# fakufaku/diffusion-separation

Hardware: AMD Instinct MI355X
Metric: separated utterances/sec (4 s, 8 kHz, 2-spk, N=30 PC steps) (higher is better)
Workload: dtype f16; 1 GPU; configs[1]: 2-spk N=30 PC sampler (+1 ald2 corrector step), batch=16 x 4.0 s @ 8 kHz per GPU and step, NCSN++ nf=64 random-init, 60 NFE/step; 4 consecutive steps (batches) in flight per GPU; batch_per_gpu=16, samples=32000, N=30, corrector_steps=1, nf=64, graph=True, batches_in_flight=4

## Files before the change

### diffusion-separation_amd/csrc/common.h

```cpp
#pragma once
#include <hip/hip_runtime.h>
#include <stdint.h>
#include <stdio.h>

#include <string>

typedef uint16_t bf16_t;
typedef __attribute__((ext_vector_type(16))) float f32x16;
typedef __attribute__((ext_vector_type(8))) __bf16 bf16x8;

#define DS_F32 0
#define DS_BF16 1
#define DS_F32_SPLIT 2
#define DS_MAX_SRC 4

void ds_set_error(const std::string& s);
#define DS_CHECK(cond, msg)                                                            \
  do {                                                                                 \
    if (!(cond)) {                                                                     \
      ds_set_error(std::string(__FILE__) + ":" + std::to_string(__LINE__) + ": " + (msg)); \
      return 1;                                                                        \
    }                                                                                  \
  } while (0)
#define DS_HIP(expr)                                                                   \
  do {                                                                                 \
    hipError_t _e = (expr);                                                            \
    if (_e != hipSuccess) {                                                            \
      ds_set_error(std::string(__FILE__) + ":" + std::to_string(__LINE__) + ": " + #expr + " -> " + \
                   hipGetErrorString(_e));                                             \
      return 1;                                                                        \
    }                                                                                  \
  } while (0)
#define DS_LAUNCH_CHECK() DS_HIP(hipGetLastError())
#define DS_FUNC_LDS_ONCE(kern, bytes)                                                                              \
  do {                                                                                                             \
    static bool done_[32] = {};                                                                                    \
    int dev_ = 0;                                                                                                  \
    (void)hipGetDevice(&dev_);                                                                                     \
    if (dev_ < 0 || dev_ >= 32 || !done_[dev_]) {                                                                  \
      DS_HIP(hipFuncSetAttribute(reinterpret_cast<const void*>(kern), hipFuncAttributeMaxDynamicSharedMemorySize, (bytes))); \
      if (dev_ >= 0 && dev_ < 32) done_[dev_] = true;                                                              \
    }                                                                                                              \
  } while (0)

typedef __attribute__((ext_vector_type(2))) float f32x2_t;
typedef __attribute__((ext_vector_type(2))) __bf16 bf16x2_t;
typedef __attribute__((ext_vector_type(2))) _Float16 f16x2_t;
typedef __attribute__((ext_vector_type(8))) _Float16 f16x8;
typedef __attribute__((ext_vector_type(4))) float f32x4_acc;
__host__ __device__ inline float bf2f(bf16_t v) {
  union { uint32_t u; float f; } c; c.u = ((uint32_t)v) << 16; return c.f;
}
__device__ inline uint32_t pack_bf16x2(float lo, float hi) {
  f32x2_t v = {lo, hi};
  return __builtin_bit_cast(uint32_t, __builtin_convertvector(v, bf16x2_t));
}
__device__ inline float bf_lo(uint32_t w) { return __uint_as_float(w << 16); }
__device__ inline float bf_hi(uint32_t w) { return __uint_as_float(w & 0xffff0000u); }
__host__ __device__ inline bf16_t f2bf(float f) {
#if defined(__HIP_DEVICE_COMPILE__)
  return __builtin_bit_cast(unsigned short, (__bf16)f);
#endif
  union { uint32_t u; float f; } c; c.f = f;
  uint32_t u = c.u;
  if ((u & 0x7fffffffu) > 0x7f800000u) return (bf16_t)((u >> 16) | 0x40u);
  u += 0x7fffu + ((u >> 16) & 1u);
  return (bf16_t)(u >> 16);
}
__device__ inline f32x16 mfma_bf32(const uint4& a, const uint4& b, const f32x16& c) {
  return __builtin_amdgcn_mfma_f32_32x32x16_bf16(__builtin_bit_cast(bf16x8, a), __builtin_bit_cast(bf16x8, b), c, 0, 0, 0);
}
__device__ inline f32x4_acc mfma_bf16(const uint4& a, const uint4& b, const f32x4_acc& c) {
  return __builtin_amdgcn_mfma_f32_16x16x32_bf16(__builtin_bit_cast(bf16x8, a), __builtin_bit_cast(bf16x8, b), c, 0, 0, 0);
}
#ifdef DS_HALF_F16
#define DS_HALF_NAME "f16"
#define DS_MFMA_H32_ASM "v_mfma_f32_32x32x16_f16"
#define DS_CVT_PK_H_ASM "v_cvt_pk_f16_f32"
#define DS_H_ONE 0x3c00u
__host__ __device__ inline float h2f(bf16_t v) { return (float)__builtin_bit_cast(_Float16, v); }
__host__ __device__ inline bf16_t f2h(float f) { return __builtin_bit_cast(unsigned short, (_Float16)f); }
__device__ inline uint32_t pack_h2(float lo, float hi) {
  f32x2_t v = {lo, hi};
  return __builtin_bit_cast(uint32_t, __builtin_convertvector(v, f16x2_t));
}
__device__ inline float h_lo(uint32_t w) { return (float)__builtin_bit_cast(f16x2_t, w)[0]; }
__device__ inline float h_hi(uint32_t w) { return (float)__builtin_bit_cast(f16x2_t, w)[1]; }
__device__ inline f32x16 mfma_h32(const uint4& a, const uint4& b, const f32x16& c) {
  return __builtin_amdgcn_mfma_f32_32x32x16_f16(__builtin_bit_cast(f16x8, a), __builtin_bit_cast(f16x8, b), c, 0, 0, 0);
}
__device__ inline f32x4_acc mfma_h16(const uint4& a, const uint4& b, const f32x4_acc& c) {
  return __builtin_amdgcn_mfma_f32_16x16x32_f16(__builtin_bit_cast(f16x8, a), __builtin_bit_cast(f16x8, b), c, 0, 0, 0);
}
#else
#define DS_HALF_NAME "bf16"
#define DS_MFMA_H32_ASM "v_mfma_f32_32x32x16_bf16"
#define DS_CVT_PK_H_ASM "v_cvt_pk_bf16_f32"
#define DS_H_ONE 0x3f80u
__host__ __device__ inline float h2f(bf16_t v) { return bf2f(v); }
__host__ __device__ inline bf16_t f2h(float f) { return f2bf(f); }
__device__ inline uint32_t pack_h2(float lo, float hi) { return pack_bf16x2(lo, hi); }
__device__ inline float h_lo(uint32_t w) { return bf_lo(w); }
__device__ inline float h_hi(uint32_t w) { return bf_hi(w); }
__device__ inline f32x16 mfma_h32(const uint4& a, const uint4& b, const f32x16& c) { return mfma_bf32(a, b, c); }
__device__ inline f32x4_acc mfma_h16(const uint4& a, const uint4& b, const f32x4_acc& c) { return mfma_bf16(a, b, c); }
#endif

template <typename T> struct Elt;
template <> struct Elt<float> {
  static constexpr int KV = 4;
  __device__ static inline float ld(const float* p) { return *p; }
  __device__ static inline void st(float* p, float v) { *p = v; }
};
template <> struct Elt<bf16_t> {
  static constexpr int KV = 8;
  __device__ static inline float ld(const bf16_t* p) { return h2f(*p); }
  __device__ static inline void st(bf16_t* p, float v) { *p = f2h(v); }
};

template <typename T> __device__ inline void load8(const T* p, float* f);
template <> __device__ inline void load8<float>(const float* p, float* f) {
  float4 a = *reinterpret_cast<const float4*>(p);
  float4 b = *reinterpret_cast<const float4*>(p + 4);
  f[0] = a.x; f[1] = a.y; f[2] = a.z; f[3] = a.w; f[4] = b.x; f[5] = b.y; f[6] = b.z; f[7] = b.w;
}
template <> __device__ inline void load8<bf16_t>(const bf16_t* p, float* f) {
  uint4 u = *reinterpret_cast<const uint4*>(p);
  f[0] = h_lo(u.x); f[1] = h_hi(u.x);
  f[2] = h_lo(u.y); f[3] = h_hi(u.y);
  f[4] = h_lo(u.z); f[5] = h_hi(u.z);
  f[6] = h_lo(u.w); f[7] = h_hi(u.w);
}
template <typename T> __device__ inline void store8(T* p, const float* f);
template <> __device__ inline void store8<float>(float* p, const float* f) {
  *reinterpret_cast<float4*>(p) = make_float4(f[0], f[1], f[2], f[3]);
  *reinterpret_cast<float4*>(p + 4) = make_float4(f[4], f[5], f[6], f[7]);
}
template <> __device__ inline void store8<bf16_t>(bf16_t* p, const float* f) {
  uint4 u;
  u.x = pack_h2(f[0], f[1]);
  u.y = pack_h2(f[2], f[3]);
  u.z = pack_h2(f[4], f[5]);
  u.w = pack_h2(f[6], f[7]);
  *reinterpret_cast<uint4*>(p) = u;
}

template <typename T> __device__ inline float exp_t(float v);
template <> __device__ inline float exp_t<float>(float v) { return expf(v); }
template <> __device__ inline float exp_t<bf16_t>(float v) { return __expf(v); }
template <typename T> __device__ inline float silu_t(float v);
template <> __device__ inline float silu_t<float>(float v) { return v / (1.0f + expf(-v)); }
template <> __device__ inline float silu_t<bf16_t>(float v) { return v * __builtin_amdgcn_rcpf(1.0f + __expf(-v)); }

__device__ inline float wave_sum(float v) {
#pragma unroll
  for (int o = 32; o > 0; o >>= 1) v += __shfl_xor(v, o, 64);
  return v;
}
__device__ inline double wave_sum_d(double v) {
#pragma unroll
  for (int o = 32; o > 0; o >>= 1) v += __shfl_xor(v, o, 64);
  return v;
}
__device__ inline float wave_max(float v) {
#pragma unroll
  for (int o = 32; o > 0; o >>= 1) v = fmaxf(v, __shfl_xor(v, o, 64));
  return v;
}

static inline int cdiv(long a, long b) { return (int)((a + b - 1) / b); }

struct ConvArgs {
  const void* x; long x_bs; int ldx;
  const void* x2; long x2_bs; int ldx2;
  int C1;
  const void* w; long w_bs;
  int w_chunked;
  const void* w_frag; const void* sw_frag;
  const void* ident_frag;
  const void* sx; long sx_bs; int ldsx;
  const void* sx2; long sx2_bs; int ldsx2; int sC1; int sCin;
  const void* sw; int sw_chunked;
  const float* gn_scale;
  const float* gn_shift; int gn_act;
  const float* bias;
  const float* bias_b; int bias_b_ld;
  int bias_mode;
  const float* div_b;
  const void* res; long res_bs; int ldr;
  float out_scale;
  void* y; long y_bs; int ldy;
  long long* stats_acc;
  const long long* gn_acc1; const long long* gn_acc2; const float* gn_gamma; const float* gn_beta;
  int gn_groups; float gn_inv_count; float gn_eps;
  int B, H, W;
  int Cin, Cout, taps;
  int dtype;
  int split;
  unsigned opts;
};
#define DS_OPT_NO_RW 1u
#define DS_OPT_NO_RW128 2u
#define DS_OPT_RW_SMALL 4u
#define DS_OPT_NO_RW_RES 8u
#define DS_OPT_NO_ATTN_FUSED 64u
#define DS_OPT_NO_SPLIT256 128u
#define DS_OPT_NO_STFT_FUSED 256u
#define DS_OPT_RW_QUARTER 1024u
#define DS_OPT_RW_BIG_HALF 2048u
#define DS_OPT_RW_HALF 512u
#define DS_OPT_NO_SW 4096u
#define DS_OPT_NO_SW_RW 8192u
#define DS_OPT_NO_SW_ROWS4 32768u
#define DS_OPT_SW_ROWS4 65536u
#define DS_OPT_NO_SWS 16384u
#define DS_OPT_NO_WFRAG 32u
unsigned ds_default_opts();
int ds_num_cus();
enum { DS_CLS_CONV_N64 = 0, DS_CLS_CONV_N32, DS_CLS_CONV_8X8, DS_CLS_GEMM_N64, DS_CLS_GEMM_N32, DS_CLS_GEMM_8X8, DS_CLS_WS,
       DS_CLS_SMALL, DS_CLS_RW, DS_CLS_ATTN, DS_CLS_SW, DS_CLS_SWS, DS_NCLS };
enum class ConvRoute { GENERIC, WS, THIN_IN, THIN_OUT, SMALL, RW, SW, SWS };
struct ConvPlan {
  ConvRoute route;
  int cls;
  int tile;
  int sw_rows;
  bool rw_ok;
  bool skip_ok;
};
ConvPlan ds_conv_plan(const ConvArgs& a);
int ds_launch_conv(const ConvArgs& a, hipStream_t st);
int ds_launch_conv(const ConvArgs& a, const ConvPlan& p, hipStream_t st);
const char* ds_last_conv_kernel();
void ds_set_last_conv_kernel(const char* name);
int ds_conv_chunk(int taps, int dtype);
__host__ __device__ inline long ds_rw_frag_index(int co, int tap, int ch, int taps, int Cout) {
  return (((((long)(ch / 64) * taps + tap) * 4 + (ch % 64) / 16) * (Cout / 32) + co / 32) * 64 + ((ch % 16) / 8) * 32 + co % 32) * 8 + ch % 8;
}
inline bool ds_rw_frag_shape(int taps, int Cin, int Cout) {
  return (Cout == 64 || Cout == 128) && (Cin == 64 || Cin == 128) && (taps == 1 || !(Cout == 128 && Cin == 64));
}
bool ds_conv_rw_supported(const ConvArgs& a);
int ds_launch_conv_rw(const ConvArgs& a, hipStream_t st);
inline bool ds_sw_frag_shape(int taps, int Cin, int Cout) { return (Cout == 64 || Cout == 128 || Cout == 256) && Cin % 64 == 0 && Cin >= 64 && Cin <= 512; }
bool ds_conv_sw_supported(const ConvArgs& a);
int ds_launch_conv_sw(const ConvArgs& a, int rows, hipStream_t st);
__host__ __device__ inline long ds_sws_frag_index(int co, int tap, int ch, int taps, int Cout, int plane) {
  return ((((((long)(ch / 32) * taps + tap) * 2 + (ch % 32) / 16) * 2 + plane) * (Cout / 32) + co / 32) * 64 + ((ch % 16) / 8) * 32 + co % 32) * 8 + ch % 8;
}
inline bool ds_sws_frag_shape(int taps, int Cin, int Cout) { return (Cout == 64 || Cout == 128 || Cout == 256) && Cin % 64 == 0 && Cin >= 64 && Cin <= 256; }
bool ds_conv_sws_supported(const ConvArgs& a);
int ds_launch_conv_sws(const ConvArgs& a, hipStream_t st);
bool ds_conv_ws_supported(const ConvArgs& a);
int ds_launch_conv_ws(const ConvArgs& a, hipStream_t st);
bool ds_conv_thin_in_supported(const ConvArgs& a);
int ds_launch_conv_thin_in(const ConvArgs& a, hipStream_t st);
bool ds_conv_thin_out_supported(const ConvArgs& a);
int ds_launch_conv_thin_out(const ConvArgs& a, hipStream_t st);
bool ds_conv_small_supported(const ConvArgs& a);
int ds_launch_conv_small(const ConvArgs& a, hipStream_t st);

struct AttnFusedArgs {
  const void* x; long x_bs; int ldx;
  const long long* gn_acc; const float* gn_gamma; const float* gn_beta; int gn_groups; float gn_inv_count; float gn_eps;
  const float* gn_scale; const float* gn_shift;
  const void* wqk; const void* wv; const void* wo;
  const float* bqk; const float* bv; const float* bo;
  void* y; long y_bs; int ldy;
  long long* stats;
  int B, L, C;
};
bool ds_attn_fused_eligible(int dtype, int channels, int L);
int ds_launch_attn_fused(const AttnFusedArgs& a, hipStream_t st);

long ds_gn_workspace_bytes(int B, int H, int W, int C);
int ds_launch_gn_stats(const void* x, int ldx, const void* x2, int ldx2, int C1, int B, int H, int W, int C, int groups,
                       float eps, const float* gamma, const float* beta, void* ws, float* scale, float* shift,
                       int dtype, hipStream_t st);
int ds_launch_gn_finalize_acc(const long long* a1, int C1, const long long* a2, int C2, int B, long npix, int groups,
                              float eps, const float* gamma, const float* beta, float* scale, float* shift,
                              hipStream_t st);
int ds_launch_gn_apply(const void* x, int ldx, const float* scale, const float* shift, int C, void* y, int ldy,
                       void* xr, int ldxr, int B, int H, int W, int act, int mode, int dtype, hipStream_t st);
int ds_launch_concat(const void* a, int lda, int Ca, const void* b, int ldb, int Cb, void* y, int ldy, long npix,
                     int dtype, hipStream_t st);
int ds_launch_softmax(const void* x, void* y, long rows, int L, int ld, int dtype, hipStream_t st);

long ds_stft_workspace_bytes(int B, int S, long T, int n_fft, int hop);
long ds_istft_workspace_bytes(int B, int S, long T, int n_fft, int hop);
int ds_launch_stft_pack(const float* xt, const float* mix, void* y, int B, int S, long T, int n_fft, int hop,
                        float exponent, float factor, int W, int Cpad, int shift, int dtype, const float* tab,
                        float* ws, hipStream_t st, int split = 0);
int ds_launch_istft(const void* x, float* out, int B, int S, long T, int n_fft, int hop, float exponent, float factor,
                    int W, int Cpad, int dtype, const float* tab, float* ws, hipStream_t st, int split = 0,
                    const float* ow = nullptr, const float* ob = nullptr, const float* tdiv = nullptr, int ow_cin = 0);
int ds_build_stft_table(int n_fft, float** dev_tab);

struct SdeP { int kind; int ndim; float d_lambda, sigma_min, sigma_max; };
__device__ inline float sde_g_of_t(const SdeP& s, float t) {
  const float r = s.sigma_max / s.sigma_min;
  return s.sigma_min * powf(r, t) * sqrtf(2.0f * logf(r));
}
__device__ inline void mix_eig(const SdeP& s, float t, float& ev1, float& ev2) {
  const float r = s.sigma_max / s.sigma_min;
  const float logsig = logf(r);
  const float mult = s.sigma_min * s.sigma_min;
  const float srp = powf(r, 2.0f * t);
  ev1 = mult * (srp - 1.0f);
  const float ex = expf(-2.0f * s.d_lambda * t);
  const float denom = 1.0f + s.d_lambda / logsig;
  ev2 = mult * (srp - ex) / denom;
}
__device__ inline void philox_round(uint32_t& c0, uint32_t& c1, uint32_t& c2, uint32_t& c3, uint32_t k0, uint32_t k1) {
  const uint64_t p0 = (uint64_t)0xD2511F53u * c0;
  const uint64_t p1 = (uint64_t)0xCD9E8D57u * c2;
  const uint32_t n0 = (uint32_t)(p1 >> 32) ^ c1 ^ k0;
  const uint32_t n1 = (uint32_t)p1;
  const uint32_t n2 = (uint32_t)(p0 >> 32) ^ c3 ^ k1;
  const uint32_t n3 = (uint32_t)p0;
  c0 = n0; c1 = n1; c2 = n2; c3 = n3;
}
__device__ inline void philox_randn4(uint64_t q, uint64_t seed, uint64_t sid, float* v) {
  uint32_t c0 = (uint32_t)q, c1 = (uint32_t)(q >> 32), c2 = (uint32_t)sid, c3 = (uint32_t)(sid >> 32);
  uint32_t k0 = (uint32_t)seed, k1 = (uint32_t)(seed >> 32);
#pragma unroll
  for (int r = 0; r < 10; ++r) {
    philox_round(c0, c1, c2, c3, k0, k1);
    k0 += 0x9E3779B9u;
    k1 += 0xBB67AE85u;
  }
  const float u0 = ((float)(c0 >> 8) + 0.5f) * (1.0f / 16777216.0f);
  const float u1 = ((float)(c1 >> 8) + 0.5f) * (1.0f / 16777216.0f);
  const float u2 = ((float)(c2 >> 8) + 0.5f) * (1.0f / 16777216.0f);
  const float u3 = ((float)(c3 >> 8) + 0.5f) * (1.0f / 16777216.0f);
  const float r0 = sqrtf(-2.0f * logf(u0)), r1 = sqrtf(-2.0f * logf(u2));
  sincosf(6.28318530718f * u1, &v[1], &v[0]);
  sincosf(6.28318530718f * u3, &v[3], &v[2]);
  v[0] *= r0; v[1] *= r0; v[2] *= r1; v[3] *= r1;
}
__device__ inline void sde_mix_drift(const SdeP& s, const float* xv, float* f, int S) {
  float mx = 0.f;
  for (int i = 0; i < S; ++i) mx += xv[i];
  mx /= (float)S;
  for (int i = 0; i < S; ++i) f[i] = -s.d_lambda * (xv[i] - mx);
}
int ds_launch_sigma_mix(const float* mix, float* out, int B, long T, int avg_len, hipStream_t st);
int ds_launch_sde_prior(const SdeP& s, const float* y, const float* z, float* x, int B, int S, long T,
                        const float* smix, hipStream_t st, const int* lens = nullptr);
int ds_launch_sde_corrector(const SdeP& s, float snr, const float* x, const float* t, const float* score,
                            const float* z, float* xo, float* xm, int B, int S, long T, const float* smix,
                            int variant, hipStream_t st, const int* lens = nullptr);
int ds_launch_sde_predictor(const SdeP& s, int N, const float* x, const float* t, const float* score, const float* z,
                            float* xo, float* xm, int B, int S, long T, const float* smix, int pflow, hipStream_t st,
                            const int* lens = nullptr);
int ds_launch_sde_coeff(const SdeP& s, const float* x, const float* t, const float* smix, float* drift,
                        float* diffusion, int B, int S, long T, float fs, float gs, hipStream_t st);
int ds_launch_sde_mean(const SdeP& s, const float* x0, const float* t, float* out, int B, int S, long T, hipStream_t st);
int ds_launch_sde_std(const SdeP& s, const float* t, const float* smix, float* L, int B, int S, long T, hipStream_t st);
int ds_launch_sde_mult_std(const float* L, const float* x, float* out, int B, int S, long T, int per_t, hipStream_t st);
int ds_launch_sde_reverse(const float* f, const float* G, const float* score, float* out, int B, long n_per_batch,
                          int g_full, int pflow, hipStream_t st);
int ds_launch_randn_batch(float* out, int B, int S, long T, const uint64_t* seeds, const int* lens, uint64_t stream_id,
                          hipStream_t st);
int ds_launch_langevin(float snr, const float* x, const float* score, const float* z, float* xo, float* xm, int B,
                       long n_per_batch, void* ws, hipStream_t st);
int ds_launch_normalize(const float* mix, float* out, float* mean, float* std, int B, long T, hipStream_t st);
int ds_launch_scale_output(const float* mix, float* sep, int B, int S, long T, hipStream_t st);
int ds_launch_randn(float* out, long n, uint64_t seed, uint64_t stream_id, hipStream_t st);
int ds_launch_gram(const float* ref, const float* est, double* out, int B, int S, long T, hipStream_t st);
int ds_launch_convert(const void* src, void* dst, long n, int sd, int dd, hipStream_t st);
int ds_launch_fill(float* p, float v, long n, hipStream_t st);

#define DS_ODE_MAX_K 7
#define DS_ODE_MAX_BLOCKS 1024
int ds_ode_tableau(int method, double* A, double* B, double* C, double* E, int* n_stages, int* error_order);
struct OdeArgs {
  SdeP s;
  const float* x; const float* score; const float* tt; float t; const float* smix;
  float* kout; int kidx; int nk;
  const float* k[DS_ODE_MAX_K]; double c[DS_ODE_MAX_K];
  double h; int mode;
  const double* y; const double* ynew; double* yo; float* xo;
  double rtol, atol; double* part;
  float* t_next_out; float t_next;
  int B, S; long T;
};
int ds_launch_ode_stage(const OdeArgs& a, hipStream_t st, int* nblk = nullptr);
int ds_launch_ode_norm_final(const double* part, int nblk, long n, double* out, hipStream_t st);
int ds_launch_ode_cast(const float* x, double* y, long n, hipStream_t st);
int ds_launch_ode_round(const double* y, float* x, long n, hipStream_t st);

int ds_launch_linear(const float* x, const float* W, const float* bias, float* y, int B, int K, int O, int silu_in,
                     hipStream_t st);
int ds_launch_linear_t(const float* x, const float* Wt, const float* bias, float* y, int B, int K, int O, int silu_in,
                       hipStream_t st);
int ds_launch_dense_transpose(const float* src, float* dst, int O, int K, int ldo, int off, hipStream_t st);
int ds_launch_fourier(const float* t, const float* Wf, float* emb, int B, int nf, hipStream_t st);
```

### diffusion-separation_amd/csrc/conv3x3_rw.hip

```cpp
#include <stdlib.h>

#ifdef RW_TIMING
#define HALO_TIMING rw
#endif
#include "conv3x3_halo.h"

namespace {

constexpr int KC = 64;
constexpr int NKB = KC / 16;
constexpr int KSC = 9 * NKB;
static_assert(KC * 2 + 16 == AROW && KC / 8 == PPL, "a pixel's chunk is one 128-byte line");

struct RwK {
  const bf16_t* x; long x_bs; int ldx; int C1;
  const bf16_t* x2; long x2_bs; int ldx2;
  const bf16_t* w; int w_chunked;
  const bf16_t* wfrag; const bf16_t* swfrag;
  const float* gn_scale; const float* gn_shift;
  const long long* gn_acc1; const long long* gn_acc2; const float* gn_gamma; const float* gn_beta;
  int gn_groups; float gn_inv_count; float gn_eps;
  const float* bias; const float* bias_b; int bias_b_ld;
  const bf16_t* res; long res_bs; int ldr;
  float out_scale;
// ... 427 lines not shown
    constexpr int LAG = ACT1 ? PIPE_LAG : 0, NUV = NU + LAG, NLU = 2 * NUV;
    constexpr int NGH = NK * RH;
    constexpr int w0 = (P == 0) ? W_E : W_N, w1 = (P == NPH - 1) ? W_E : W_N, CAP = NGH * (w0 + w1);
    auto lub = [](int GP) constexpr { return NLU * (GP <= NGH ? GP * w0 : NGH * w0 + (GP - NGH) * w1) / CAP; };
    constexpr int NLE = RH * 22;
    constexpr int R0 = HF * RH, ER0 = HF ? 0 : RH;
    const char* fb = sA + slot_r * LDS_A + fbase + R0 * HW_ * AROW;
#ifndef RW_BUILTIN_MFMA
    if constexpr (EPI) {
#pragma unroll
      for (int r = 0; r < RH; ++r) asm volatile("s_nop 11" : "+v"(acc[ER0 + r]));
    }
#endif
    if constexpr (HF == 0 && C1 < NCH) act_tab(C1);
    constexpr int SUB = CONV ? 3 : 1, RFN = CONV ? RH + 2 : RH, NG = NK / SUB;
    static_assert(SUB * RH >= RFN, "the next group's fragments are read in the MFMA slots of the current one");
    auto ldg = [&](int g, int j) __attribute__((always_inline)) {
      const int dx = CONV ? g / NKB : 1, kb = g % NKB, row = CONV ? j : j + 1;
      return *reinterpret_cast<const u32x4_t*>(fb + (row * HW_ + dx) * AROW + kb * 32);
    };
    u32x4_t rf[2][RFN];
#pragma unroll
    for (int j = 0; j < RFN; ++j) rf[0][j] = ldg(0, j);
    auto widx = [](int ks) {
      if (!CONV) return ks;
      const int g = ks / 3, dy = ks % 3, dx = g / NKB, kb = g % NKB;
      return (dy * 3 + dx) * NKB + kb;
    };
#define RW_FRAG(ks, r) rf[((ks) / SUB) & 1][(r) + (CONV ? (ks) % SUB : 0)]
#define RW_FRAG_LAST(ks) rf[((ks) / SUB) & 1][RFN - 1]
    u32x4_t wl = {0, 0, 0, 0}, wln = {0, 0, 0, 0};
    if constexpr (W0 + widx(0) >= NWR) wl = *reinterpret_cast<const u32x4_t*>(sWl + (W0 + widx(0) - NWR) * G::WL_STEP);
    int rels[2][NL];
    auto fetch_rels = [&](int ks, int par) __attribute__((always_inline)) {
      const int gp0 = HF * NGH + ks * RH;
#pragma unroll
      for (int L = lub(gp0); L < lub(gp0 + RH); ++L) {
        const int u = (L >> 1) - LAG;
        if ((L & 1) && u >= 0 && u < NU && (u & 3) == 3 && (u >> 2) >= NI)
          rels[par][u >> 2] = REL_REGS ? relreg[(u >> 2) - NI] : sDesc[((u >> 2) - NI) * NT + tid];
      }
    };
    fetch_rels(0, 0);

    auto unit_lump = [&](int L, int par) __attribute__((always_inline)) {
      const int v = L >> 1;
      const int u0 = v < NU ? v : -1, u1 = LAG ? ((v >= 1 && v - 1 < NU) ? v - 1 : -1) : v, u2 = v - LAG;
      const bool s2 = u2 >= 0 && u2 < NU;
      if ((L & 1) == 0) {
        if constexpr (ACT1 && ACT_PK) {
          if (u0 >= 0) {
            asm volatile("v_pk_fma_f16 %0, %1, %2, %3" : "=v"(uzp[u0 % 3]) : "v"(pa[u0 >> 2][u0 & 3]), "v"(psc[u0 & 3]), "v"(psh[u0 & 3]));
            if constexpr (MODE == 2 && !FOLD) asm volatile("v_pk_mul_f16 %0, %1, %2" : "=v"(uxp[u0 % 3]) : "v"(uzp[u0 % 3]), "s"(0xbdc5bdc5u));
          }
          if constexpr (MODE == 2) {
            if (u1 >= 0) asm volatile("v_pk_add_f16 %0, %1, %2" : "=v"(udp[u1 % 3]) : "v"(utp[u1 % 3]), "s"(0x3c003c00u));
            if (s2) asm volatile("v_pk_mul_f16 %0, %1, %2" : "=v"(so[u2 & 3]) : "v"(uzp[u2 % 3]), "v"(urp[u2 % 3]));
            if (u0 >= 0) asm volatile("v_exp_f16 %0, %1" : "=v"(utp[u0 % 3]) : "v"(FOLD ? uzp[u0 % 3] : uxp[u0 % 3]));
            if (u1 >= 0) asm volatile("v_rcp_f16 %0, %1" : "=v"(urp[u1 % 3]) : "v"(udp[u1 % 3]));
          } else {
            if (s2) so[u2 & 3] = uzp[u2 % 3];
          }
        } else if constexpr (ACT1) {
          if (u0 >= 0) unit_s01(std::integral_constant<int, C1>{}, u0, -1);
        }
      } else {
        if constexpr (ACT1 && ACT_PK) {
          if constexpr (MODE == 2) {
            if (u0 >= 0) asm volatile("v_exp_f16_sdwa %0, %1 dst_sel:WORD_1 dst_unused:UNUSED_PRESERVE src0_sel:WORD_1" : "+v"(utp[u0 % 3]) : "v"(FOLD ? uzp[u0 % 3] : uxp[u0 % 3]));
            if (u1 >= 0) asm volatile("v_rcp_f16_sdwa %0, %1 dst_sel:WORD_1 dst_unused:UNUSED_PRESERVE src0_sel:WORD_1" : "+v"(urp[u1 % 3]) : "v"(udp[u1 % 3]));
          }
        } else if constexpr (ACT1) {
          if (u1 >= 0) unit_s01(std::integral_constant<int, C1>{}, -1, u1);
        }
#ifndef RW_ABL_NOSTAGE
        if (s2) {
          const int rel = ((u2 & 3) == 3 && (u2 >> 2) >= NI) ? rels[par][u2 >> 2] : 0;
          if constexpr (ACT1 && ACT_PK) unit_fin(std::integral_constant<int, C1>{}, std::integral_constant<int, C2>{}, g1, g2, slot_r ^ 1, u2, rel);
          else unit_s2(std::integral_constant<int, C1>{}, std::integral_constant<int, C2>{}, g1, g2, slot_r ^ 1, u2, rel);
        }
#endif
      }
    };
    auto epi_lump = [&](int LE) __attribute__((always_inline)) {
      const int rr = ER0 + LE / 22, x = LE % 22;
      if (x < 20) {
        const int j = x / 10, y = x % 10;
        const bool isA = y == 0 || y == 1 || y == 3 || y == 5 || y == 7;
        const int pr = y == 0 ? 0 : (y == 1 ? 1 : (y == 2 ? 0 : (y == 3 ? 2 : (y == 4 ? 1 : (y == 5 ? 3 : (y == 6 ? 2 : (y == 7 ? 4 : 3)))))));
        if (y == 9) {
          if (j == 0) {
            asm volatile("v_permlane32_swap_b32 %0, %1" : "+v"(osa[0]), "+v"(osa[2]));
            asm volatile("v_permlane32_swap_b32 %0, %1" : "+v"(osa[1]), "+v"(osa[3]));
          } else {
            asm volatile("v_permlane32_swap_b32 %0, %1" : "+v"(osb[0]), "+v"(osb[2]));
            asm volatile("v_permlane32_swap_b32 %0, %1" : "+v"(osb[1]), "+v"(osb[3]));
          }
        } else if (isA) {
          if (pr < 4) {
            const int e0 = 8 * j + 2 * pr;
            const float b0 = pr == 0 ? breg[j][0].x : (pr == 1 ? breg[j][0].z : (pr == 2 ? breg[j][1].x : breg[j][1].z));
            const float b1 = pr == 0 ? breg[j][0].y : (pr == 1 ? breg[j][0].w : (pr == 2 ? breg[j][1].y : breg[j][1].w));
            asm volatile("v_fma_f32 %0, %1, %2, %3" : "=v"(et[pr & 1][0]) : "v"(acc[rr][e0]), "s"(osc), "v"(b0));
            asm volatile("v_fma_f32 %0, %1, %2, %3" : "=v"(et[pr & 1][1]) : "v"(acc[rr][e0 + 1]), "s"(osc), "v"(b1));
          }
          if (pr >= 1) {
            const int q = pr - 1;
            if (j == 0) asm volatile(DS_CVT_PK_H_ASM " %0, %1, %2" : "=v"(osa[q]) : "v"(et[q & 1][0]), "v"(et[q & 1][1]));
            else asm volatile(DS_CVT_PK_H_ASM " %0, %1, %2" : "=v"(osb[q]) : "v"(et[q & 1][0]), "v"(et[q & 1][1]));
          }
        } else {
#ifndef RW_ABL_NOSTATS
          const int e0 = 8 * j + 2 * pr;
          asm volatile("v_add_f32 %0, %0, %1" : "+v"(ssum[e0]) : "v"(et[pr & 1][0]));
          asm volatile("v_add_f32 %0, %0, %1" : "+v"(ssum[e0 + 1]) : "v"(et[pr & 1][1]));
          asm volatile("v_fma_f32 %0, %1, %1, %0" : "+v"(ssq[e0]) : "v"(et[pr & 1][0]));
          asm volatile("v_fma_f32 %0, %1, %1, %0" : "+v"(ssq[e0 + 1]) : "v"(et[pr & 1][1]));
#endif
        }
      } else if (x == 20) {
#pragma unroll
        for (int d = 0; d < 4; ++d) asm volatile("v_permlane16_swap_b32 %0, %1" : "+v"(osa[d]), "+v"(osb[d]));
      } else {
        const int pix = ge.pix0 + (pg * RPW + rr) * p.W + (lane & 15);
        const unsigned o = __umul24((unsigned)pix, (unsigned)p.ldy * 2u) + spiece;
#ifdef RW_TIMING
        const unsigned o1 = (p.dbg & 1) ? OOB : o, o2 = (p.dbg & 1) ? OOB : o + 16u * (unsigned)p.ldy * 2u;
#else
        const unsigned o1 = o, o2 = o + 16u * (unsigned)p.ldy * 2u;
#endif
#ifdef RW_ABL_NOSTORE
        asm volatile("" :: "v"(osa), "v"(osb), "v"(o1), "v"(o2));
#else
        __builtin_amdgcn_raw_buffer_store_b128(osa, ry, o1, 0, 0);
        __builtin_amdgcn_raw_buffer_store_b128(osb, ry, o2, 0, 0);
#endif
      }
    };

#pragma unroll
    for (int ks = 0; ks < NK; ++ks) {
      if (ks + 1 < NK) fetch_rels(ks + 1, (ks + 1) & 1);
      const int wi = W0 + widx(ks), win = W0 + widx(ks + 1 < NK ? ks + 1 : ks);
      if (win >= NWR && ks + 1 < NK) wln = *reinterpret_cast<const u32x4_t*>(sWl + (win - NWR) * G::WL_STEP);
      const u32x4_t wk = wi < NWR ? wf[wi < NWR ? wi : 0] : wl;
#define RW_DEP , "v"(RW_FRAG_LAST(ks))
#pragma unroll
      for (int r = 0; r < RH; ++r) {
        if (wi < NWR) {
          if (P == 0 && ks == 0) asm volatile(DS_MFMA_H32_ASM " %0, %1, %2, 0" : "=v"(acc[R0 + r]) : "a"(wk), "v"(RW_FRAG(ks, r)) RW_DEP);
          else asm volatile(DS_MFMA_H32_ASM " %0, %1, %2, %0" : "+v"(acc[R0 + r]) : "a"(wk), "v"(RW_FRAG(ks, r)) RW_DEP);
        } else {
          if (P == 0 && ks == 0) asm volatile(DS_MFMA_H32_ASM " %0, %1, %2, 0" : "=v"(acc[R0 + r]) : "v"(wk), "v"(RW_FRAG(ks, r)) RW_DEP);
          else asm volatile(DS_MFMA_H32_ASM " %0, %1, %2, %0" : "+v"(acc[R0 + r]) : "v"(wk), "v"(RW_FRAG(ks, r)) RW_DEP);
        }
        {
          const int g = ks / SUB, q = (ks % SUB) * RH + r;
          if (q < RFN && g + 1 < NG) rf[(g + 1) & 1][q] = ldg(g + 1, q);
        }
        const int gh = ks * RH + r, gp = HF * NGH + gh;
#pragma unroll
        for (int L = lub(gp); L < lub(gp + 1); ++L) unit_lump(L, ks & 1);
#ifndef RW_ABL_NOEPI
        if constexpr (EPI) {
#pragma unroll
          for (int LE = gh * NLE / NGH; LE < (gh + 1) * NLE / NGH; ++LE) epi_lump(LE);
        }
#endif
      }
      wl = wln;
      __builtin_amdgcn_sched_barrier(0);
    }
  };

  TileG gc = tile_geom(0);
  constexpr int CH0 = G::chunk_of(0), CH1 = G::chunk_of(1 % NPH);
  const TileG g1st = NPH > 1 ? gc : tile_geom(1);
  {
#pragma unroll
    for (int k = 0; k < NL; ++k) issue_one(std::integral_constant<int, CH0>{}, gc, k, k < NI ? 0 : sDesc[(k < NI ? 0 : k - NI) * NT + tid]);
    load_weights();
    build_tables();
    sync_lds();
    RT_MARK(7)
    if constexpr (REL_REGS) {
#pragma unroll
      for (int k = 0; k < NB; ++k) relreg[k] = sDesc[k * NT + tid];
    }
    if constexpr (BIAS_REGS) {
#pragma unroll
      for (int j = 0; j < 2; ++j) {
        breg[j][0] = *reinterpret_cast<const float4*>(sTab + 2 * CIN + cg * 32 + 8 * (2 * j) + 4 * h);
        breg[j][1] = *reinterpret_cast<const float4*>(sTab + 2 * CIN + cg * 32 + 8 * (2 * j + 1) + 4 * h);
      }
    }
    act_tab(CH0);
#pragma unroll
    for (int u = 0; u < NL * 4; ++u)
      unit(std::integral_constant<int, CH0>{}, std::integral_constant<int, CH1>{}, gc, g1st, 0, u,
           (u >> 2) < NI ? 0 : sDesc[((u >> 2) < NI ? 0 : (u >> 2) - NI) * NT + tid]);
  }
  RT_MARK(0)
  TileG gp = tile_geom(nt);
  int ph = 0;
  TileG gnc = tile_geom(1);
  int ty2 = (t0 + 2) / p.tiles_x, tx2 = (t0 + 2) - ty2 * p.tiles_x;
  for (int i = 0; i < nt; ++i) {
    const TileG gn = gnc, gnn = geom_at(ty2, tx2, i + 2 < nt);
    auto run = [&](auto self, auto P_) __attribute__((always_inline)) {
      constexpr int P = decltype(P_)::value;
      sync_lds();
      RT_MARK(1)
      const int slot_r = ph & 1;
      half(P_, std::integral_constant<int, 0>{}, std::integral_constant<bool, P == 0>{}, slot_r, gp, ((P + 1) / NPH == 0 ? gc : gn), ((P + 2) / NPH == 0 ? gc : ((P + 2) / NPH == 1 ? gn : gnn)));
      if constexpr (P == 0) {
        if (i == 0) {
#pragma unroll
          for (int j = 0; j < 16; ++j) { ssum[j] = 0.f; ssq[j] = 0.f; }
        }
      }
      half(P_, std::integral_constant<int, 1>{}, std::integral_constant<bool, P == NPH - 1>{}, slot_r, gc, ((P + 1) / NPH == 0 ? gc : gn), ((P + 2) / NPH == 0 ? gc : ((P + 2) / NPH == 1 ? gn : gnn)));
      ++ph;
      RT_MARK(G::chunk_of(P) < NCH ? 2 : 3)
      if constexpr (P + 1 < NPH) self(self, std::integral_constant<int, P + 1>{});
    };
    run(run, std::integral_constant<int, 0>{});
    gp = gc;
    gc = gn;
    gnc = gnn;
    if (++tx2 == p.tiles_x) { tx2 = 0; ++ty2; }
  }
#ifndef RW_BUILTIN_MFMA
#pragma unroll
  for (int r = 0; r < RH; ++r) asm volatile("s_nop 11" : "+v"(acc[RH + r]));
#endif
#pragma unroll
  for (int e = 0; e < RH * 2; ++e) {
    float4 t0, t1;
    epi_bias(e & 1, t0, t1);
    epi_unit(gp, RH + (e >> 1), e & 1, t0, t1);
  }
  RT_MARK(4)
  if (has_stats) {
    __syncthreads();
    float* red = reinterpret_cast<float*>(smem);
    constexpr int RED_ROW = 36;
#pragma unroll
    for (int q = 0; q < 4; ++q) {
      *reinterpret_cast<float4*>(red + tid * RED_ROW + 4 * q) = make_float4(ssum[4 * q], ssum[4 * q + 1], ssum[4 * q + 2], ssum[4 * q + 3]);
      *reinterpret_cast<float4*>(red + tid * RED_ROW + 16 + 4 * q) = make_float4(ssq[4 * q], ssq[4 * q + 1], ssq[4 * q + 2], ssq[4 * q + 3]);
    }
    __syncthreads();
    if (tid < 2 * CO) {
      const int co = tid >> 1, st = tid & 1;
      const int wcg = co >> 5, c32 = co & 31, q = c32 >> 3, hh = (c32 >> 2) & 1, i = c32 & 3;
      double a = 0.0;
      for (int wpg = 0; wpg < PGN; ++wpg)
        for (int l = 0; l < 32; ++l) {
          const int t = (wpg * NCG + wcg) * 64 + hh * 32 + l;
          a += (double)red[t * RED_ROW + st * 16 + 4 * q + i];
        }
      ds_stat_flush(p.stats + ((long)b * CO + co) * 2, st, a);
    }
  }
  RT_MARK(5)
  RT_FLUSH
}

int rw_blocks_per_image(const ConvArgs& a, int tiles) {
  int g = ds_num_cus() / a.B;
#ifdef RW_TIMING
  if (getenv("DIFFSEP_RW_G")) g = atoi(getenv("DIFFSEP_RW_G"));
#endif
  if ((a.opts & DS_OPT_RW_HALF) && g >= 2 && tiles / g <= 4) g /= 2;
  if ((a.opts & DS_OPT_RW_QUARTER) && g >= 4 && tiles / g <= 4) g /= 4;
  if ((a.opts & DS_OPT_RW_BIG_HALF) && g >= 2 && tiles / g > 4) g /= 2;
  if (g < 1) g = 1;
  if (g > tiles) g = tiles;
  return g;
}

template <int NCH, int RPW, int NSK, int MODE, int NCG>
int rw_launch(const RwK& k0, const ConvArgs& a, hipStream_t st) {
  using G = RwGeom<NCH, RPW, NSK, NCG>;
  RwK k = k0;
  const int tiles = (a.H / G::TH) * (a.W / TW);
  k.G = rw_blocks_per_image(a, tiles);
  k.tiles_x = a.W / TW;
  k.tiles_per_img = tiles;
  auto kern = conv3x3_rw_kernel<NCH, RPW, NSK, MODE, NCG>;
  DS_FUNC_LDS_ONCE(kern, G::LDS_TOTAL);
  hipLaunchKernelGGL(kern, dim3(a.B * k.G), dim3(NT), G::LDS_TOTAL, st, k);
  DS_LAUNCH_CHECK();
  {
    static char name[64] = {0};
    if (!name[0]) snprintf(name, sizeof(name), "conv3x3_rw_kernel<%d,%d,%d,%d,%d>", NCH, RPW, NSK, MODE, NCG);
    ds_set_last_conv_kernel(name);
  }
  return 0;
}

}

bool ds_conv_rw_supported(const ConvArgs& a) {
  const int CO = a.Cout;
  if (!(a.dtype == DS_BF16 && a.taps == 9 && ((CO == 64 && (a.Cin == 64 || a.Cin == 128)) || (CO == 128 && a.Cin == 128)) &&
        a.w_bs == 0 && (a.w_chunked == 0 || a.w_chunked == 32) && a.bias_mode == 0 && !a.div_b && a.W % TW == 0 && a.H % 8 == 0 &&
        a.H >= 32 && a.W >= 32 && a.ldy >= CO && a.ldy % 8 == 0 && (!a.res || (a.ldr >= CO && a.ldr % 8 == 0))))
    return false;
  if (a.x2 ? !(a.C1 % KC == 0 && a.C1 > 0 && a.C1 < a.Cin && a.ldx % 8 == 0 && a.ldx2 % 8 == 0) : a.ldx % 8 != 0) return false;
  const bool gn = a.gn_scale || a.gn_acc1;
  if (gn && !a.gn_act) return false;
  if (a.gn_acc1 && !(a.gn_groups > 0 && a.Cin % a.gn_groups == 0 && a.Cin / a.gn_groups <= 8 && (!a.x2 || a.gn_acc2))) return false;
  if (a.sx) {
    if (!(a.sw && !a.res && (a.sCin == 64 || a.sCin == 128 || (a.sCin == 192 && CO == 64 && a.Cin == 64)) && a.ldsx % 8 == 0 &&
          (!a.sx2 || (a.sC1 % KC == 0 && a.sC1 > 0 && a.sC1 < a.sCin && a.ldsx2 % 8 == 0)) &&
          (a.sw_chunked == 0 || ((a.sw_chunked & (a.sw_chunked - 1)) == 0 && a.sw_chunked >= 16))))
      return false;
    if (a.Cin == 128 && CO == 64) return false;
  }
  if (a.res && a.Cin == 128 && CO == 64) return false;
  if (CO == 128 && (a.sx || a.res) && !gn) return false;
  return true;
}

int ds_launch_conv_rw(const ConvArgs& a, hipStream_t st) {
  RwK k;
  k.x = reinterpret_cast<const bf16_t*>(a.x); k.x_bs = a.x_bs; k.ldx = a.ldx; k.C1 = a.x2 ? a.C1 : a.Cin;
  k.x2 = reinterpret_cast<const bf16_t*>(a.x2); k.x2_bs = a.x2_bs; k.ldx2 = a.x2 ? a.ldx2 : a.ldx;
  k.w = reinterpret_cast<const bf16_t*>(a.w); k.w_chunked = a.w_chunked;
  k.wfrag = reinterpret_cast<const bf16_t*>(a.w_frag);
  k.swfrag = (a.sx && a.sw) ? reinterpret_cast<const bf16_t*>(a.sw_frag) : nullptr;
  k.gn_scale = a.gn_scale; k.gn_shift = a.gn_shift;
  k.gn_acc1 = a.gn_acc1; k.gn_acc2 = a.gn_acc2; k.gn_gamma = a.gn_gamma; k.gn_beta = a.gn_beta;
  k.gn_groups = a.gn_groups; k.gn_inv_count = a.gn_inv_count; k.gn_eps = a.gn_eps;
  k.bias = a.bias; k.bias_b = a.bias_b; k.bias_b_ld = a.bias_b_ld;
  k.res = reinterpret_cast<const bf16_t*>(a.res); k.res_bs = a.res_bs; k.ldr = a.ldr;
  k.out_scale = a.out_scale;
  k.y = reinterpret_cast<bf16_t*>(a.y); k.y_bs = a.y_bs; k.ldy = a.ldy;
  k.stats = a.stats_acc;
  k.sx = reinterpret_cast<const bf16_t*>(a.sx); k.sx_bs = a.sx_bs; k.ldsx = a.ldsx; k.sC1 = a.sx2 ? a.sC1 : a.sCin;
  k.sx2 = reinterpret_cast<const bf16_t*>(a.sx2); k.sx2_bs = a.sx2_bs; k.ldsx2 = a.sx2 ? a.ldsx2 : a.ldsx;
  k.sw = reinterpret_cast<const bf16_t*>(a.sw); k.sw_chunked = a.sw_chunked; k.sw_shift = a.sw_chunked ? __builtin_ctz(a.sw_chunked) : 0;
  k.sCin = a.sCin;
  k.H = a.H; k.W = a.W; k.G = 0; k.tiles_x = 0; k.tiles_per_img = 0;
#ifdef RW_TIMING
  k.dbg = getenv("DIFFSEP_RW_DBG") ? atoi(getenv("DIFFSEP_RW_DBG")) : 0;
#else
  k.dbg = 0;
#endif
  if (a.res) {
    k.sx = reinterpret_cast<const bf16_t*>(a.res); k.sx_bs = a.res_bs; k.ldsx = a.ldr; k.sC1 = a.Cout;
    k.sx2 = nullptr; k.sx2_bs = 0; k.ldsx2 = a.ldr; k.sw = nullptr; k.sw_chunked = 0; k.sw_shift = 0; k.sCin = a.Cout;
  }
  const int mode = ((a.gn_scale || a.gn_acc1) && a.gn_act) ? 2 : 0;
  const int nsk = a.sx ? a.sCin / KC : (a.res ? a.Cout / KC : 0);
  if (a.Cout == 128) {
    if (mode == 0) return rw_launch<2, 4, 0, 0, 4>(k, a, st);
    if (nsk == 0) return rw_launch<2, 4, 0, 2, 4>(k, a, st);
    if (nsk == 1) return rw_launch<2, 4, 1, 2, 4>(k, a, st);
    return rw_launch<2, 4, 2, 2, 4>(k, a, st);
  }
#define RW_GO(NCH_, NSK_) return mode == 2 ? rw_launch<NCH_, 4, NSK_, 2, 2>(k, a, st) : rw_launch<NCH_, 4, NSK_, 0, 2>(k, a, st)
  if (a.Cin == 128) RW_GO(2, 0);
  if (nsk == 0) RW_GO(1, 0);
  if (nsk == 1) RW_GO(1, 1);
  if (nsk == 2) RW_GO(1, 2);
  RW_GO(1, 3);
#undef RW_GO
}
```

### diffusion-separation_amd/csrc/conv_mfma.hip

```cpp
#include <stdlib.h>
#include <string.h>

#include <type_traits>

#include "conv_device.h"

#ifdef CONV_TIMING
__device__ unsigned long long g_conv_dbg[16];
#define CT_DECL unsigned long long ct_prev = __builtin_readcyclecounter(), ct_acc[12] = {0, 0, 0, 0, 0, 0, 0, 0, 0, 0, 0, 0};
#define CT_MARK(i) { unsigned long long ct_now = __builtin_readcyclecounter(); ct_acc[i] += ct_now - ct_prev; ct_prev = ct_now; }
#define CT_WAIT __builtin_amdgcn_s_waitcnt(0);
#define CT_FLUSH if (threadIdx.x == 0) { for (int q = 0; q < 12; ++q) atomicAdd(&g_conv_dbg[q], ct_acc[q]); atomicAdd(&g_conv_dbg[15], 1ull); }
extern "C" int diffsep_debug_read(unsigned long long* out, int reset) {
  (void)hipMemcpyFromSymbol(out, HIP_SYMBOL(g_conv_dbg), sizeof(unsigned long long) * 16);
  if (reset) { unsigned long long z[16] = {0}; (void)hipMemcpyToSymbol(HIP_SYMBOL(g_conv_dbg), z, sizeof(z)); }
  return 0;
}
#else
#define CT_DECL
#define CT_MARK(i)
#define CT_WAIT
#define CT_FLUSH
#endif

// ... 474 lines not shown
      } else {
        if (c + 1 < ncht) load_chunk(c + 1);
        CT_MARK(5)
        mma_chunk(std::false_type{}, std::false_type{});
      }
      CT_MARK(6)
    }
    if constexpr (SKIP_OK) {
      for (int c = nch; c < ncht; ++c) {
        __syncthreads();
        write_chunk(true);
        __syncthreads();
        if (c + 1 < ncht) load_chunk(c + 1);
        mma_chunk(std::false_type{}, std::true_type{});
      }
    }
  };
  if (!has_gn) run_chunks(std::integral_constant<int, 0>{});
  else if (p.gn_act) run_chunks(std::integral_constant<int, 2>{});
  else run_chunks(std::integral_constant<int, 1>{});

  const __amdgpu_buffer_rsrc_t ry =
      rsrc(reinterpret_cast<T*>(p.y) + (long)b * p.y_bs, (unsigned)M * p.ldy * ESZ);
  const __amdgpu_buffer_rsrc_t rr = rsrc(
      p.res ? reinterpret_cast<const T*>(p.res) + (long)b * p.res_bs : reinterpret_cast<const T*>(p.y),
      p.res ? (unsigned)M * p.ldr * ESZ : 0u);
#ifdef ABL_NOEPI
  {
    float t = 0.f;
#pragma unroll
    for (int i = 0; i < WM; ++i)
#pragma unroll
      for (int j = 0; j < WN; ++j)
#pragma unroll
        for (int r = 0; r < 16; ++r) t += acc[i][j][r];
    if (t == 12345.678f) reinterpret_cast<float*>(p.y)[tid] = t;
    return;
  }
#endif
  const int cout8 = (p.Cout + 7) & ~7;
  const float dvs = p.div_b ? p.div_b[b] : 1.0f;
  constexpr int NCG = BN / 8;
  static_assert(NT % NCG == 0, "a thread keeps one cout group across the epilogue loop");
  constexpr int WME = WM / EP;
  constexpr int RV = ESZ * 8 / 16;
  const int cg = tid % NCG;
  const int co = n0 + cg * 8;
  float bv[8];
  {
    float b1[8], b2[8];
    const float* pb1 = (p.bias_mode == 0 && p.bias) ? p.bias : nullptr;
    const float* pb2 = (p.bias_mode == 0 && p.bias_b) ? p.bias_b + (long)b * p.bias_b_ld : nullptr;
#pragma unroll
    for (int j = 0; j < 8; ++j) {
      const int cc = (co + j < p.Cout) ? co + j : p.Cout - 1;
      b1[j] = pb1 ? pb1[cc] : 0.f;
      b2[j] = pb2 ? pb2[cc] : 0.f;
    }
#pragma unroll
    for (int j = 0; j < 8; ++j) bv[j] = (co + j < p.Cout) ? b1[j] + b2[j] : 0.f;
#pragma unroll
    for (int j = 0; j < 8; ++j) asm volatile("" : "+v"(bv[j]));
  }
  const bool overhang = (TAPS == 9) ? (y0 + TH > p.H || x0 + TW > p.W) : (m0 + BM > M);
  const bool lean = p.bias_mode == 0 && !p.div_b && !overhang && n0 + BN <= cout8;
  float ssum[8], ssq[8];
#pragma unroll
  for (int j = 0; j < 8; ++j) { ssum[j] = 0.f; ssq[j] = 0.f; }
#pragma unroll
  for (int e = 0; e < EP; ++e) {
    __syncthreads();
#pragma unroll
    for (int i = 0; i < WME; ++i)
#pragma unroll
      for (int j = 0; j < WN; ++j)
#pragma unroll
        for (int g = 0; g < 4; ++g) {
          const int lp = (wm * WME + i) * 32 + l32;
          const int cc = (wn * WN + j) * 32 + 8 * g + 4 * h;
          *reinterpret_cast<float4*>(smem + lp * OROW + cc * 4) =
              make_float4(acc[e * WME + i][j][4 * g], acc[e * WME + i][j][4 * g + 1], acc[e * WME + i][j][4 * g + 2],
                          acc[e * WME + i][j][4 * g + 3]);
        }
    constexpr int NROW = (BM / EP) / (NT / NCG);
    static_assert((BM / EP) % (NT / NCG) == 0, "whole rows per thread");
    int mrow[NROW];
    unsigned voy[NROW], vor[NROW];
    uint4 rraw[NROW][RV];
    constexpr int RSTEP = NT / NCG;
    const int pp0 = tid / NCG;
    const int gy0 = y0 + pp0 / TW, gx0 = x0 + pp0 % TW;
    const int mlin0 = (TAPS == 9) ? gy0 * p.W + gx0 : m0 + pp0;
    const int mstep = (TAPS == 9) ? (RSTEP / TW) * p.W : RSTEP;
    const bool col_ok = co < cout8 && (TAPS != 9 || gx0 < p.W);
#pragma unroll
    for (int it = 0; it < NROW; ++it) {
      int m = -1;
      if (EP == 1 && (TAPS != 9 || RSTEP % TW == 0)) {
        const bool ok = col_ok && ((TAPS == 9) ? (gy0 + it * (RSTEP / TW) < p.H) : (mlin0 + it * mstep < M));
        m = ok ? mlin0 + it * mstep : -1;
      } else {
        const int lp = tid / NCG + it * (NT / NCG);
        const int pp = ((lp / (32 * WME)) * WM + e * WME + (lp / 32) % WME) * 32 + (lp & 31);
        if (TAPS == 9) {
          const int gy = y0 + pp / TW, gx = x0 + pp % TW;
          if (gy < p.H && gx < p.W) m = gy * p.W + gx;
        } else {
          if (m0 + pp < M) m = m0 + pp;
        }
        if (co >= cout8) m = -1;
      }
      mrow[it] = m;
      voy[it] = m >= 0 ? (unsigned)(m * p.ldy + co) * ESZ : OOB;
      vor[it] = m >= 0 ? (unsigned)(m * p.ldr + co) * ESZ : OOB;
#pragma unroll
      for (int q = 0; q < RV; ++q) rraw[it][q] = ld16(rr, vor[it], 16u * q);
    }
    __syncthreads();
    CT_MARK(7)
    uint4 oraw[NROW][RV];
    if (lean) {
      const float osc = p.out_scale;
      float bs[8];
#pragma unroll
      for (int j = 0; j < 8; ++j) bs[j] = bv[j] * osc;
      const bool has_res = p.res != nullptr, has_stats = p.stats != nullptr;
#pragma unroll
      for (int it = 0; it < NROW; ++it) {
        const int lp = tid / NCG + it * (NT / NCG);
        const float4 a0 = *reinterpret_cast<const float4*>(smem + lp * OROW + cg * 32);
        const float4 a1 = *reinterpret_cast<const float4*>(smem + lp * OROW + cg * 32 + 16);
        float v[8] = {a0.x, a0.y, a0.z, a0.w, a1.x, a1.y, a1.z, a1.w};
#pragma unroll
        for (int j = 0; j < 8; ++j) v[j] = fmaf(v[j], osc, bs[j]);
        if (has_res) {
          float rv[8];
          unpack8<T>(rraw[it], rv);
#pragma unroll
          for (int j = 0; j < 8; ++j) v[j] = fmaf(rv[j], osc, v[j]);
        }
        if (has_stats) {
#pragma unroll
          for (int j = 0; j < 8; ++j) {
            ssum[j] += v[j];
            ssq[j] = fmaf(v[j], v[j], ssq[j]);
          }
        }
        pack8<T>(v, oraw[it]);
      }
    } else {
#pragma unroll
      for (int it = 0; it < NROW; ++it) {
        const int m = mrow[it];
        const int lp = tid / NCG + it * (NT / NCG);
        float v[8];
        const float4 a0 = *reinterpret_cast<const float4*>(smem + lp * OROW + cg * 32);
        const float4 a1 = *reinterpret_cast<const float4*>(smem + lp * OROW + cg * 32 + 16);
        v[0] = a0.x; v[1] = a0.y; v[2] = a0.z; v[3] = a0.w; v[4] = a1.x; v[5] = a1.y; v[6] = a1.z; v[7] = a1.w;
        float rv[8];
        unpack8<T>(rraw[it], rv);
        if (p.div_b) {
#pragma unroll
          for (int j = 0; j < 8; ++j) v[j] = v[j] / dvs;
        }
        if (p.bias_mode == 1 && p.bias) {
          const float rowb = p.bias[m < 0 ? 0 : m];
#pragma unroll
          for (int j = 0; j < 8; ++j) v[j] = (co + j < p.Cout) ? v[j] + rowb : 0.f;
        }
#pragma unroll
        for (int j = 0; j < 8; ++j) v[j] = (v[j] + bv[j] + rv[j]) * p.out_scale;
        const float keep = m < 0 ? 0.f : 1.f;
#pragma unroll
        for (int j = 0; j < 8; ++j) {
          ssum[j] = fmaf(keep, v[j], ssum[j]);
          asm volatile("" : "+v"(ssum[j]));
          ssq[j] = fmaf(keep * v[j], v[j], ssq[j]);
          asm volatile("" : "+v"(ssq[j]));
        }
        pack8<T>(v, oraw[it]);
      }
    }
    CT_MARK(8)
#pragma unroll
    for (int it = 0; it < NROW; ++it)
#pragma unroll
      for (int q = 0; q < RV; ++q) buf_store16(ry, voy[it], 16u * q, oraw[it][q]);
    CT_MARK(9)
  }
  if (p.stats) {
    __syncthreads();
    float* sr = reinterpret_cast<float*>(smem);
    const int r = tid / NCG;
#pragma unroll
    for (int j = 0; j < 8; ++j) {
      sr[(r * BN + cg * 8 + j) * 2 + 0] = ssum[j];
      sr[(r * BN + cg * 8 + j) * 2 + 1] = ssq[j];
    }
    __syncthreads();
    if (tid < BN && n0 + tid < p.Cout) {
      double a = 0.0, q = 0.0;
      for (int rr2 = 0; rr2 < NT / NCG; ++rr2) {
        a += (double)sr[(rr2 * BN + tid) * 2 + 0];
        q += (double)sr[(rr2 * BN + tid) * 2 + 1];
      }
      long long* o = p.stats + ((long)b * p.Cout + n0 + tid) * 2;
      ds_stat_add(o, (long long)llrint(a * DS_STAT_SUM_SCALE));
      ds_stat_add(o + 1, (long long)llrint(q * DS_STAT_SQ_SCALE));
    }
  }
  CT_MARK(10)
  CT_FLUSH
}

template <typename T, int TAPS, int TH, int TW, int BN, int WM, int WN, int KC, int EP = 1, int OCC = 2, int SP = 0, int NT = 256>
static int launch_cfg(const ConvArgs& a, hipStream_t st) {
  using G = ConvGeom<T, TAPS, TH, TW, BN, KC, EP, NT>;
  constexpr int LDS = G::LDS + 4096;
  auto kern = conv_mfma_kernel<T, TAPS, TH, TW, BN, WM, WN, KC, EP, OCC, SP, NT>;
  DS_FUNC_LDS_ONCE(kern, LDS);
  ConvK k;
  k.x = a.x; k.x_bs = a.x_bs; k.ldx = a.ldx; k.C1 = a.x2 ? a.C1 : a.Cin;
  k.x2 = a.x2; k.x2_bs = a.x2_bs; k.ldx2 = a.ldx2;
  k.w = a.w; k.w_bs = a.w_bs;
  DS_CHECK(a.w_chunked == 0 || (a.w_chunked >= 8 && KC % a.w_chunked == 0 && a.Cin % KC == 0 && (!a.x2 || a.C1 % KC == 0)),
           "conv: chunk-major weights need kc | the kernel's chunk width and whole chunks per source");
  k.w_chunked = a.w_chunked; k.w_shift = a.w_chunked ? __builtin_ctz(a.w_chunked) : 0;
  DS_CHECK((a.w_chunked & (a.w_chunked - 1)) == 0 && (a.sw_chunked & (a.sw_chunked - 1)) == 0, "conv: weight chunks are powers of two");
  DS_CHECK(!a.sx || (G::SKIP_OK && a.sw && a.sCin % 8 == 0 && a.ldsx % 8 == 0 &&
                     (a.sw_chunked == 0 || (a.sw_chunked >= 8 && KC % a.sw_chunked == 0 && a.sCin % KC == 0 &&
                                            (!a.sx2 || a.sC1 % KC == 0)))),
           "conv: bad fused skip convolution arguments");
  k.sx = a.sx; k.sx_bs = a.sx_bs; k.ldsx = a.ldsx; k.sx2 = a.sx2; k.sx2_bs = a.sx2_bs; k.ldsx2 = a.ldsx2;
  k.sC1 = a.sx2 ? a.sC1 : a.sCin; k.sCin = a.sCin; k.sw = a.sw; k.sw_chunked = a.sw_chunked; k.sw_shift = a.sw_chunked ? __builtin_ctz(a.sw_chunked) : 0;
  k.gn_scale = a.gn_scale; k.gn_shift = a.gn_shift; k.gn_act = a.gn_act;
  k.bias = a.bias; k.bias_b = a.bias_b; k.bias_b_ld = a.bias_b_ld; k.bias_mode = a.bias_mode; k.div_b = a.div_b;
  k.res = a.res; k.res_bs = a.res_bs; k.ldr = a.ldr; k.out_scale = a.out_scale;
  k.y = a.y; k.y_bs = a.y_bs; k.ldy = a.ldy; k.stats = a.stats_acc;
  k.gn_acc1 = a.gn_acc1; k.gn_acc2 = a.gn_acc2; k.gn_gamma = a.gn_gamma; k.gn_beta = a.gn_beta;
  k.gn_groups = a.gn_groups; k.gn_inv_count = a.gn_inv_count; k.gn_eps = a.gn_eps;
  DS_CHECK(!a.gn_acc1 || (a.Cin <= 512 && a.gn_groups > 0 && a.Cin % a.gn_groups == 0 && (!a.x2 || a.gn_acc2)),
           "conv: bad GroupNorm accumulator arguments");
  k.H = a.H; k.W = a.W; k.Cin = a.Cin; k.Cout = a.Cout;
  dim3 grid;
  if (TAPS == 9) {
    k.tiles_x = cdiv(a.W, TW);
    grid.x = k.tiles_x * cdiv(a.H, TH);
  } else {
    k.tiles_x = 1;
    grid.x = cdiv((long)a.H * a.W, TH * TW);
  }
  grid.y = cdiv(a.Cout, BN);
  grid.z = a.B;
  hipLaunchKernelGGL(kern, grid, dim3(NT), LDS, st, k);
  DS_LAUNCH_CHECK();
  {
    static char name[128] = {0};
    if (!name[0])
      snprintf(name, sizeof(name), "conv_mfma_kernel<%s,%d,%d,%d,%d,%d,%d,%d,%d,%d,%d,%d>", sizeof(T) == 2 ? DS_HALF_NAME : "float", TAPS,
               TH, TW, BN, WM, WN, KC, EP, OCC, SP, NT);
    ds_set_last_conv_kernel(name);
  }
  return 0;
}

static thread_local const char* g_last_conv_kernel = "";
const char* ds_last_conv_kernel() { return g_last_conv_kernel; }
void ds_set_last_conv_kernel(const char* name) { g_last_conv_kernel = name; }

template <typename T, int SP = 0>
static int launch_typed(const ConvArgs& a, int tile, hipStream_t st) {
  constexpr int KC9 = (sizeof(T) == 4) ? 16 : 32;
  constexpr int KC1 = (sizeof(T) == 4) ? 32 : 64;
  switch (tile) {
    case DS_CLS_CONV_N64: {
      const long blocks = (long)cdiv(a.W, 32) * cdiv(a.H, 8) * cdiv(a.Cout, 64) * a.B;
      if constexpr (sizeof(T) == 2) {
      if (blocks <= 128) return launch_cfg<T, 9, 8, 16, 64, 1, 2, KC9, 1, 2, SP>(a, st);
      if (!a.sx && a.Cin >= 128 && a.Cout == 64 && a.H % 16 == 0 && blocks >= 1024)
        return launch_cfg<T, 9, 16, 32, 64, 2, 2, KC9, 2, 2, SP, 512>(a, st);
      if (a.Cout % 128 == 0 && blocks >= 1024)
        return launch_cfg<T, 9, 8, 32, 128, 2, 2, KC9, 2, 2, SP, 512>(a, st);
      }
      return launch_cfg<T, 9, 8, 32, 64, 2, 2, KC9, 1, 2, SP>(a, st);
    }
    case DS_CLS_CONV_N32: return launch_cfg<T, 9, 8, 32, 32, 2, 1, KC9, 1, 2, SP>(a, st);
    case DS_CLS_CONV_8X8: {
      const bool deep = a.Cin % (2 * KC9) == 0 && (!a.x2 || a.C1 % (2 * KC9) == 0) &&
                        (!a.sx || (a.sCin % (2 * KC9) == 0 && (!a.sx2 || a.sC1 % (2 * KC9) == 0)));
      if (deep) return launch_cfg<T, 9, 8, 8, 64, 1, 1, KC9 * 2, 1, 2, SP>(a, st);
      return launch_cfg<T, 9, 8, 8, 64, 1, 1, KC9, 1, 2, SP>(a, st);
    }
    case DS_CLS_GEMM_N64: return launch_cfg<T, 1, 8, 32, 64, 2, 2, KC1, 1, 2, SP>(a, st);
    case DS_CLS_GEMM_N32: return launch_cfg<T, 1, 8, 32, 32, 2, 1, KC1, 1, 2, SP>(a, st);
    default: return launch_cfg<T, 1, 8, 8, 64, 1, 1, KC1, 1, 2, SP>(a, st);
  }
}

int ds_conv_chunk(int taps, int dtype) {
  if (dtype == DS_F32) return taps == 9 ? 16 : 32;
  return taps == 9 ? 32 : 64;
}

ConvPlan ds_conv_plan(const ConvArgs& a) {
  const unsigned o = a.opts;
  const bool any_size = o & DS_OPT_RW_SMALL;
  const long cus = ds_num_cus(), ncb = a.Cout >= 128 ? a.Cout / 128 : 1;
  const long t8 = (long)a.B * (a.H / 8) * (a.W / 32) * ncb, t4 = (long)a.B * (a.H / 4) * (a.W / 32) * ncb;
  ConvPlan p = {ConvRoute::GENERIC, -1, -1, 0, false, false};
  auto routed = [&](ConvRoute r, int cls) {
    p.route = r; p.cls = cls; p.tile = r == ConvRoute::GENERIC ? cls : -1; p.skip_ok = a.taps == 9 && cls != DS_CLS_CONV_N32;
    return p;
  };
  if (!(o & DS_OPT_NO_SWS) && ds_conv_sws_supported(a) && (2 * (a.Cout == 64 ? t8 : t4) >= cus || any_size))
    return routed(ConvRoute::SWS, DS_CLS_SWS);
  p.rw_ok = !(o & DS_OPT_NO_RW) && ds_conv_rw_supported(a) &&
            (a.Cout == 128 ? !(o & DS_OPT_NO_RW128) && (t4 >= cus || any_size)
                           : !(a.res && (o & DS_OPT_NO_RW_RES)) && (t8 >= cus || any_size));
  if (ds_conv_sw_supported(a)) {
    const bool rows8 = a.H % 8 == 0 && !(o & DS_OPT_SW_ROWS4);
    const int rows = a.Cout == 64 ? 4 : rows8 && (t4 >= 2 * cus || any_size) ? 8 : (2 * t4 >= cus || any_size) ? 4 : 0;
    p.sw_rows = rows ? rows : (rows8 ? 8 : 4);
    const bool take = a.Cout == 64 ? t8 >= cus || any_size
                                   : rows && !(rows == 4 && (o & DS_OPT_NO_SW_ROWS4)) && (!p.rw_ok || (!(o & DS_OPT_NO_SW_RW) && t8 < 2 * cus));
    if (take && !(o & DS_OPT_NO_SW)) return routed(ConvRoute::SW, DS_CLS_SW);
  }
  if (p.rw_ok) return routed(ConvRoute::RW, DS_CLS_RW);
  if (ds_conv_ws_supported(a)) return routed(ConvRoute::WS, DS_CLS_WS);
  if (ds_conv_thin_in_supported(a)) return routed(ConvRoute::THIN_IN, DS_CLS_WS);
  if (ds_conv_thin_out_supported(a)) return routed(ConvRoute::THIN_OUT, DS_CLS_WS);
  if (ds_conv_small_supported(a)) return routed(ConvRoute::SMALL, DS_CLS_SMALL);
  if (a.taps == 9)
    return routed(ConvRoute::GENERIC, !(a.W >= 32 && a.H >= 8) ? DS_CLS_CONV_8X8 : a.Cout <= 32 ? DS_CLS_CONV_N32 : DS_CLS_CONV_N64);
  if ((long)a.H * a.W >= 1024 || ((long)a.H * a.W >= 256 && a.Cout >= 1024))
    return routed(ConvRoute::GENERIC, a.Cout <= 32 ? DS_CLS_GEMM_N32 : DS_CLS_GEMM_N64);
  return routed(ConvRoute::GENERIC, DS_CLS_GEMM_8X8);
}

int ds_launch_conv(const ConvArgs& a, hipStream_t st) { return ds_launch_conv(a, ds_conv_plan(a), st); }
int ds_launch_conv(const ConvArgs& a, const ConvPlan& p, hipStream_t st) {
  DS_CHECK(a.taps == 1 || a.taps == 9, "conv: taps must be 1 or 9");
  DS_CHECK(a.Cin % 8 == 0 && a.ldx % 8 == 0, "conv: Cin and ldx must be multiples of 8");
  DS_CHECK(a.B > 0 && a.H > 0 && a.W > 0 && a.Cout > 0, "conv: empty problem");
  DS_CHECK(a.x && a.w && a.y, "conv: null pointer");
  DS_CHECK(a.ldy >= ((a.Cout + 7) & ~7), "conv: output pixel stride must cover Cout rounded up to 8");
  DS_CHECK(!a.x2 || (a.C1 % 8 == 0 && a.C1 > 0 && a.C1 < a.Cin && a.ldx2 % 8 == 0), "conv: bad concat split");
  {
    const long esz = a.dtype == DS_F32 ? 4 : 2, M = (long)a.H * a.W;
    long mld = a.ldx > a.ldy ? a.ldx : a.ldy;
    if (a.x2 && a.ldx2 > mld) mld = a.ldx2;
    if (a.res && a.ldr > mld) mld = a.ldr;
    DS_CHECK(M * mld * esz < 2147483647L, "conv: image too large for 32-bit buffer offsets");
    DS_CHECK((long)a.Cout * a.taps * a.Cin * esz < 2147483647L, "conv: weight tensor too large");
  }
  switch (p.route) {
    case ConvRoute::SWS: return ds_launch_conv_sws(a, st);
    case ConvRoute::SW: return ds_launch_conv_sw(a, p.sw_rows, st);
    case ConvRoute::RW: return ds_launch_conv_rw(a, st);
    case ConvRoute::WS: return ds_launch_conv_ws(a, st);
    case ConvRoute::THIN_IN: return ds_launch_conv_thin_in(a, st);
    case ConvRoute::THIN_OUT: return ds_launch_conv_thin_out(a, st);
    case ConvRoute::SMALL: return ds_launch_conv_small(a, st);
    case ConvRoute::GENERIC: break;
  }
  if (a.dtype == DS_F32) return a.split ? launch_typed<float, 1>(a, p.tile, st) : launch_typed<float, 0>(a, p.tile, st);
  if (a.dtype == DS_BF16) return launch_typed<bf16_t>(a, p.tile, st);
  DS_CHECK(false, "conv: unknown dtype");
}
```

### diffusion-separation_amd/csrc/engine.hip

```cpp
#include "engine_host.h"

static thread_local std::string g_err;
void ds_set_error(const std::string& s) { g_err = s; }
extern "C" const char* diffsep_last_error(void) { return g_err.c_str(); }
extern "C" const char* diffsep_version(void) {
#ifdef DS_HALF_F16
    return "diffsep-hip 0.3 (gfx950, 16-bit storage f16)";
#else
    return "diffsep-hip 0.3 (gfx950, 16-bit storage bf16)";
#endif
}

static const struct { const char* name; const char* env; unsigned bit; } kOpts[] = {
    {"no_rw", "DIFFSEP_NO_RW", DS_OPT_NO_RW},
    {"no_rw128", "DIFFSEP_NO_RW128", DS_OPT_NO_RW128},
    {"rw_small", "DIFFSEP_RW_SMALL", DS_OPT_RW_SMALL},
    {"no_rw_res", "DIFFSEP_NO_RW_RES", DS_OPT_NO_RW_RES},
    {"no_wfrag", nullptr, DS_OPT_NO_WFRAG},
    {"no_attn_fused", nullptr, DS_OPT_NO_ATTN_FUSED},
    {"no_stft_fused", "DIFFSEP_NO_STFT_FUSED", DS_OPT_NO_STFT_FUSED},
    {"rw_half", "DIFFSEP_RW_HALF", DS_OPT_RW_HALF},
    {"rw_quarter", "DIFFSEP_RW_QUARTER", DS_OPT_RW_QUARTER},
    {"rw_big_half", "DIFFSEP_RW_BIG_HALF", DS_OPT_RW_BIG_HALF},
    {"no_split256", nullptr, DS_OPT_NO_SPLIT256},
    {"no_sw", "DIFFSEP_NO_SW", DS_OPT_NO_SW},
    {"no_sws", "DIFFSEP_NO_SWS", DS_OPT_NO_SWS},
    {"no_sw_rows4", "DIFFSEP_NO_SW_ROWS4", DS_OPT_NO_SW_ROWS4},
    {"sw_rows4", nullptr, DS_OPT_SW_ROWS4},
    {"no_sw_rw", "DIFFSEP_NO_SW_RW", DS_OPT_NO_SW_RW}};
static std::atomic<unsigned> g_opts{0};
static std::once_flag g_opts_once;
unsigned ds_default_opts() {
  std::call_once(g_opts_once, [] {
    for (const auto& o : kOpts) {
      const char* v = o.env ? getenv(o.env) : nullptr;
      if (v && *v && strcmp(v, "0") != 0) g_opts |= o.bit;
    }
  });
  return g_opts;
}
int ds_num_cus() {
  static std::atomic<int> cus[32];
  int dev = 0;
  if (hipGetDevice(&dev) != hipSuccess || dev < 0 || dev >= 32) dev = 0;
  int c = cus[dev].load(std::memory_order_relaxed);
  if (c <= 0) {
    hipDeviceProp_t prop;
    c = hipGetDeviceProperties(&prop, dev) == hipSuccess ? prop.multiProcessorCount : 0;
    if (c <= 0) c = 256;
    cus[dev].store(c, std::memory_order_relaxed);
  }
  return c;
}
static int opt_bit(const char* name, unsigned* bit) {
  for (const auto& o : kOpts)
    if (!strcmp(name, o.name)) { *bit = o.bit; return 0; }
  return 1;
}
extern "C" int32_t diffsep_set_option(const char* name, int64_t value) {
  DS_CHECK(name, "set_option: null name");
  unsigned bit = 0;
  if (opt_bit(name, &bit)) { ds_set_error(std::string("set_option: unknown option '") + name + "'"); return 1; }
  ds_default_opts();
  if (value) g_opts.fetch_or(bit); else g_opts.fetch_and(~bit);
  return 0;
}

static Tn cat_view(const Tn& a, const Tn& b) {
  Tn t = a;
  t.C = a.C + b.C; t.C1 = a.C; t.p2 = b.p; t.ld2 = b.ld;
  t.sa2 = b.sa;
  return t;
}

static void* e_alloc(diffsep_engine* e, size_t bytes) {
  const size_t a = (e->top + 255) & ~(size_t)255;
  e->top = a + bytes;
  if (e->dry) return (void*)(uintptr_t)(a + 256);
  if (e->dbg_alloc) fprintf(stderr, "[diffsep alloc] %zu %zu\n", a, bytes);
  return e->arena + a;
}
static long long* e_alloc_stats(diffsep_engine* e, size_t bytes) {
  const size_t a = (e->stats_used + 255) & ~(size_t)255;
  e->stats_used = a + bytes;
  if (e->dry) { if (e->stats_used > e->stats_need) e->stats_need = e->stats_used; return (long long*)(uintptr_t)256; }
  if (e->stats_used > e->stats_need) { ds_set_error("internal: GroupNorm accumulator region overflow"); return nullptr; }
  return (long long*)(e->stats_ptr + a);
}
int stats_begin(diffsep_engine* e, hipStream_t st) {
  e->stats_used = 0;
  if (e->dry) { e->stats_need = 0; return 0; }
  e->stats_ptr = (char*)e_alloc(e, e->stats_need);
  if (e->stats_need && ds_launch_fill((float*)e->stats_ptr, 0.f, (long)(e->stats_need / 4), st)) return 1;
  return 0;
}
static Tn e_tensor(diffsep_engine* e, int B, int H, int W, int C) {
  Tn t;
  t.C = C; t.ld = C; t.H = H; t.W = W;
  t.p = e_alloc(e, (size_t)B * H * W * C * e->esz);
  if (e->track_tensors && !e->dry) e->tracked.push_back({t.p, (long)B * H * W * C, H, W, C});
  return t;
}
float* e_f32(diffsep_engine* e, size_t n) { return (float*)e_alloc(e, n * 4); }
static const float* P(diffsep_engine* e, const PRef& r) { return e->d_blob + r.off; }
static const void* PK(diffsep_engine* e, long off) { return e->d_pack + off * e->esz; }
static const void* PKF(diffsep_engine* e, long off) { return off >= 0 ? e->d_pack + off * e->esz : nullptr; }

static bool ablated(const diffsep_engine* e, int H) {
  if (!e->ablate) return false;
  const unsigned bit = H <= 16 ? 1u : H == 32 ? 2u : H == 64 ? 4u : H == 128 ? 32u : H == 256 ? 64u : 0u;
  return (e->ablate & bit) != 0;
}

struct GnAff {
  float* scale = nullptr; float* shift = nullptr;
  const long long* acc1 = nullptr; const long long* acc2 = nullptr;
  const float* gamma = nullptr; const float* beta = nullptr; int groups = 0; float inv_count = 0.f;
};
struct SkipConv { const Tn* x; const void* w; int chunk; const void* w_frag; };
struct Conv {
  const Tn& x;
  const void* w;
  int Cout, taps;
  Conv(const Tn& x_, const void* w_, int Cout_, int taps_) : x(x_), w(w_), Cout(Cout_), taps(taps_) {}
  const void* w_frag = nullptr;
  const void* ident_frag = nullptr;
  const float* bias = nullptr;
  const float* bias_b = nullptr;
  int bias_b_ld = 0;
  const float* div_b = nullptr;
  const Tn* res = nullptr;
  float scale = 1.f;
  const GnAff* gn = nullptr;
  const SkipConv* skip = nullptr;
  bool want_stats = false;
};
static ConvArgs conv_args(const diffsep_engine* e, const Conv& c, const Tn& y, int B) {
  const Tn& x = c.x;
  ConvArgs a;
  memset(&a, 0, sizeof(a));
  a.B = B; a.Cout = c.Cout; a.taps = c.taps; a.dtype = e->cfg.dtype; a.split = e->split; a.opts = e->opts;
  conv_input(a, x);
  if (c.gn) {
    a.gn_scale = c.gn->scale; a.gn_shift = c.gn->shift; a.gn_act = 1;
    if (c.gn->acc1) {
      a.gn_acc1 = c.gn->acc1; a.gn_acc2 = c.gn->acc2; a.gn_gamma = c.gn->gamma; a.gn_beta = c.gn->beta;
      a.gn_groups = c.gn->groups; a.gn_inv_count = c.gn->inv_count; a.gn_eps = 1e-6f;
    }
  }
  a.w = c.w; a.w_bs = 0; a.w_chunked = weight_chunk(c.taps, x.C, x.p2 ? x.C1 : 0, e->cfg.dtype);
  const bool use_frag = (e->cfg.dtype == DS_BF16 || (e->cfg.dtype == DS_F32 && e->split)) && !(e->opts & DS_OPT_NO_WFRAG);
  a.w_frag = use_frag ? c.w_frag : nullptr;
  a.ident_frag = use_frag ? c.ident_frag : nullptr;
  a.bias = c.bias; a.bias_b = c.bias_b; a.bias_b_ld = c.bias_b_ld; a.bias_mode = 0; a.div_b = c.div_b;
  if (c.res) conv_residual(a, *c.res);
  a.out_scale = c.scale;
  conv_output(a, y);
  if (c.skip) {
    conv_skip_input(a, *c.skip->x);
    a.sw = c.skip->w; a.sw_chunked = c.skip->chunk;
    a.sw_frag = use_frag ? c.skip->w_frag : nullptr;
  }
  return a;
}
static int conv(diffsep_engine* e, const Conv& c, Tn& y, int B, hipStream_t st) {
  ConvArgs a = conv_args(e, c, y, B);
  if (c.want_stats) {
    y.sa = e_alloc_stats(e, (size_t)B * c.Cout * 2 * sizeof(long long));
    if (!y.sa) return 1;
    a.stats_acc = y.sa;
  }
  const ConvPlan p = ds_conv_plan(a);
  DS_CHECK(!a.sx || p.skip_ok, "internal: fused skip conv on an unsupported tile");
  if (c.want_stats && e->dbg_alloc && !e->dry)
    fprintf(stderr, "[diffsep stats] %ld Cin %d Cout %d taps %d HxW %dx%d res %d skip %d bias_b %d cfg %d\n",
            (long)((char*)y.sa - e->stats_ptr), a.Cin, c.Cout, c.taps, a.H, a.W, c.res != nullptr, c.skip != nullptr,
            c.bias_b != nullptr, p.cls);
  if (e->dry || ablated(e, a.H)) return 0;
  if (!e->prof) return ds_launch_conv(a, p, st);
  diffsep_engine::ProfRec r;
  r.flops = 2.0 * ((double)a.taps * a.Cin + (a.sx ? a.sCin : 0)) * a.Cout * (double)a.H * a.W * a.B;
  {
    const double esz = a.dtype == DS_F32 ? 4.0 : 2.0;
    r.bytes = esz * ((double)a.B * a.H * a.W *
                         ((double)a.Cin + a.Cout + (a.res ? a.Cout : 0) + (a.sx ? a.sCin : 0)) +
                     ((double)a.taps * a.Cin + (a.sx ? a.sCin : 0)) * a.Cout);
  }
  r.cls = p.cls;
  r.B = a.B; r.H = a.H; r.W = a.W; r.Cin = a.Cin; r.Cout = a.Cout; r.taps = a.taps; r.sCin = a.sx ? a.sCin : 0; r.res = a.res != nullptr;
  const int rc = prof_launch(e, st, r, [&]() { return ds_launch_conv(a, p, st); });
  e->prof_recs.back().kernel = ds_last_conv_kernel();
  return rc;
}

static int gn_stats(diffsep_engine* e, const Tn& x, const float* gamma, const float* beta, int B, GnAff& aff,
                    hipStream_t st, bool lazy = false) {
  const int groups = gn_group_count(x.C);
  aff = GnAff();
  const bool have_acc = x.sa && (!x.p2 || x.sa2);
  if (have_acc && lazy && x.C <= 512) {
    aff.acc1 = x.sa; aff.acc2 = x.sa2; aff.gamma = gamma; aff.beta = beta; aff.groups = groups;
    aff.inv_count = gn_inv_count((long)x.H * x.W, x.C, groups);
    return 0;
  }
  aff.scale = e_f32(e, (size_t)B * x.C);
  aff.shift = e_f32(e, (size_t)B * x.C);
  if (have_acc) {
    if (e->dry || (e->ablate & 16u)) return 0;
    return ds_launch_gn_finalize_acc(x.sa, x.p2 ? x.C1 : x.C, x.sa2, x.p2 ? x.C - x.C1 : 0, B, (long)x.H * x.W, groups,
                                     1e-6f, gamma, beta, aff.scale, aff.shift, st);
  }
  void* ws = e_alloc(e, (size_t)ds_gn_workspace_bytes(B, x.H, x.W, x.C));
  if (e->dry) return 0;
  return ds_launch_gn_stats(x.p, x.ld, x.p2, x.ld2, x.C1, B, x.H, x.W, x.C, groups, 1e-6f, gamma, beta, ws, aff.scale,
                            aff.shift, e->cfg.dtype, st);
}
static int gn_apply(diffsep_engine* e, const Tn& x, const GnAff* aff, const Tn* y, const Tn* xr, int B, int act,
                    int mode, hipStream_t st) {
  if (e->dry || (e->ablate & 8u)) return 0;
  const double esz = e->cfg.dtype == DS_F32 ? 4.0 : 2.0, nin = (double)B * x.H * x.W * x.C;
  const double fo = mode == 1 ? 4.0 : (mode == 2 ? 0.25 : 1.0);
  const double bytes = esz * nin * (1.0 + fo * ((y ? 1 : 0) + (xr ? 1 : 0)));
  const char* name = mode == 1 ? (aff ? "gn_fir_up (GroupNorm + SiLU + FIR x2 up of act and raw)" : "fir_up (pyramid)")
                               : (mode == 2 ? (aff ? "gn_fir_down (GroupNorm + SiLU + FIR x2 down of act and raw)" : "fir_down (pyramid)")
                                            : "gn_apply (GroupNorm affine + SiLU)");
  return prof_launch(e, st, hbm_rec(name, bytes, B, x.H, x.W, x.C), [&]() {
    return ds_launch_gn_apply(x.p, x.ld, aff ? aff->scale : nullptr, aff ? aff->shift : nullptr, x.C, y ? y->p : nullptr,
                              y ? y->ld : 0, xr ? xr->p : nullptr, xr ? xr->ld : 0, B, x.H, x.W, act, mode, e->cfg.dtype,
                              st);
  });
}

static const float kInvSqrt2 = 0.70710678118654752440f;

static int conv1_folded_skip(diffsep_engine* e, const Module& m, const Tn& h1, const Tn& skip_src, const GnAff& a1, Tn& out,
                             int B, hipStream_t st) {
  const SkipConv sk = {&skip_src, PK(e, m.pk2), weight_chunk(9, m.in_ch, m.in_c1, e->cfg.dtype), PKF(e, m.pf2)};
  Conv c(h1, PK(e, m.pk1), m.out_ch, 9);
  c.w_frag = PKF(e, m.pf1); c.gn = &a1; c.skip = &sk; c.scale = kInvSqrt2; c.want_stats = true;
  c.bias = P(e, m.conv1_b); c.bias_b = P(e, m.conv2_b);
  return conv(e, c, out, B, st);
}

int res_block(diffsep_engine* e, const Module& m, const Tn& x, const float* temb_proj, int B, Tn& out,
              hipStream_t st) {
  DS_CHECK(x.C == m.in_ch, "internal: resblock channel mismatch");
  const int mode = m.up ? 1 : (m.down ? 2 : 0);
  const int Ho = m.up ? 2 * x.H : (m.down ? x.H / 2 : x.H);
  const int Wo = m.up ? 2 * x.W : (m.down ? x.W / 2 : x.W);
  GnAff a0, a1;
  const float* temb = temb_proj + m.temb_off;
  if (e->cfg.dtype == DS_BF16 && mode == 0 && x.p2 && m.pf0a >= 0 && x.C1 == 128 && x.sa && x.sa2 &&
      x.H >= ((e->opts & DS_OPT_NO_SW) ? 128 : 256) && !(e->opts & (DS_OPT_NO_SPLIT256 | DS_OPT_NO_WFRAG))) {
    Tn xa = x, xb = x;
    xa.C = 128; xa.p2 = nullptr; xa.C1 = 0; xa.ld2 = 0; xa.sa2 = nullptr;
    xb.p = x.p2; xb.ld = x.ld2; xb.C = 128; xb.p2 = nullptr; xb.C1 = 0; xb.ld2 = 0; xb.sa = x.sa2; xb.sa2 = nullptr;
    GnAff ga, gb;
    ga.acc1 = xa.sa; ga.gamma = P(e, m.gn0_w); ga.beta = P(e, m.gn0_b);
    ga.groups = gn_group_count(x.C) / 2;
    ga.inv_count = gn_inv_count((long)x.H * x.W, x.C, gn_group_count(x.C));
    gb = ga; gb.acc1 = xb.sa; gb.gamma = ga.gamma + 128; gb.beta = ga.beta + 128;
    Conv c0a(xa, PK(e, m.pk0), m.out_ch, 9);
    c0a.w_frag = PKF(e, m.pf0a); c0a.gn = &ga; c0a.bias = P(e, m.conv0_b); c0a.bias_b = temb; c0a.bias_b_ld = e->arch.dense_total;
    Tn h1p; h1p.C = h1p.ld = m.out_ch; h1p.H = Ho; h1p.W = Wo;
    ConvArgs half = conv_args(e, c0a, h1p, B); half.opts &= ~DS_OPT_RW_SMALL;
    if (ds_conv_plan(half).rw_ok) {
      h1p = e_tensor(e, B, Ho, Wo, m.out_ch);
      Tn h1 = e_tensor(e, B, Ho, Wo, m.out_ch);
      const long half0 = 4L * 9 * m.out_ch * 32;
      if (conv(e, c0a, h1p, B, st)) return 1;
      Conv c0b(xb, PK(e, m.pk0 + half0), m.out_ch, 9);
      c0b.w_frag = PKF(e, m.pf0b); c0b.gn = &gb; c0b.res = &h1p; c0b.want_stats = true;
      if (conv(e, c0b, h1, B, st)) return 1;
      if (gn_stats(e, h1, P(e, m.gn1_w), P(e, m.gn1_b), B, a1, st, true)) return 1;
      out = e_tensor(e, B, Ho, Wo, m.out_ch);
      if (!(e->opts & DS_OPT_NO_SW) && m.pf2 >= 0) return conv1_folded_skip(e, m, h1, x, a1, out, B, st);
      Tn outp = e_tensor(e, B, Ho, Wo, m.out_ch);
      const SkipConv sk = {&xa, PK(e, m.pk2), weight_chunk(9, 128, 0, e->cfg.dtype), PKF(e, m.pf2a)};
      Conv c1(h1, PK(e, m.pk1), m.out_ch, 9);
      c1.w_frag = PKF(e, m.pf1); c1.gn = &a1; c1.skip = &sk; c1.bias = P(e, m.conv1_b); c1.bias_b = P(e, m.conv2_b);
      if (conv(e, c1, outp, B, st)) return 1;
      Conv c2b(xb, PK(e, m.pk2b), m.out_ch, 1);
      c2b.res = &outp; c2b.scale = kInvSqrt2; c2b.want_stats = true;
      return conv(e, c2b, out, B, st);
    }
  }
  if (gn_stats(e, x, P(e, m.gn0_w), P(e, m.gn0_b), B, a0, st, mode == 0)) return 1;
  Tn h1 = e_tensor(e, B, Ho, Wo, m.out_ch);
  Tn xr = x, h0m;
  if (mode) {
    DS_CHECK(x.p2 == nullptr, "internal: resampling block on a concat view");
    h0m = e_tensor(e, B, Ho, Wo, m.in_ch);
    xr = e_tensor(e, B, Ho, Wo, m.in_ch);
    if (gn_apply(e, x, &a0, &h0m, &xr, B, 1, mode, st)) return 1;
  }
  if (!m.has_conv2) DS_CHECK(xr.p2 == nullptr, "internal: identity skip on a concat view");
  Conv c0(mode ? h0m : x, PK(e, m.pk0), m.out_ch, 9);
  c0.w_frag = PKF(e, m.pf0); c0.gn = mode ? nullptr : &a0; c0.want_stats = true;
  c0.bias = P(e, m.conv0_b); c0.bias_b = temb; c0.bias_b_ld = e->arch.dense_total;
  if (conv(e, c0, h1, B, st)) return 1;
  if (gn_stats(e, h1, P(e, m.gn1_w), P(e, m.gn1_b), B, a1, st, true)) return 1;
  out = e_tensor(e, B, Ho, Wo, m.out_ch);
  if (m.has_conv2 && fuse_skip(m)) return conv1_folded_skip(e, m, h1, xr, a1, out, B, st);
  Tn skip = xr;
  if (m.has_conv2) {
    skip = e_tensor(e, B, Ho, Wo, m.out_ch);
    Conv c2(xr, PK(e, m.pk2), m.out_ch, 1);
    c2.bias = P(e, m.conv2_b);
    if (conv(e, c2, skip, B, st)) return 1;
  }
  Conv c1(h1, PK(e, m.pk1), m.out_ch, 9);
  c1.w_frag = PKF(e, m.pf1); c1.ident_frag = m.has_conv2 ? nullptr : PKF(e, m.pf_id);
  c1.gn = &a1; c1.bias = P(e, m.conv1_b); c1.res = &skip; c1.scale = kInvSqrt2; c1.want_stats = true;
  return conv(e, c1, out, B, st);
}

int attention_core(const Tn& q, const void* k, const void* vt, const Tn& o, int B, void* scores, void* probs, int dtype,
                   hipStream_t st, int split) {
  const int L = q.W, C = q.C, Lp = rup8(L);
  Tn s = q, p = q;
// ... 552 lines not shown
```

Baseline: 76.02 utterances/s.

## Add 512-thread RW2 conv3x3 kernel variant and widen RW eligibility to short images

Adds a new 64->64 channel 3x3 convolution kernel (RW2) that uses 512 threads per block. It stages eight-row tiles and splits weight fragments between registers and LDS. The kernel is wired into the conv planner behind an off-by-default flag, so it only runs when the rw2_all option is set. Separately, the existing RW kernel now accepts Cout=64 layers with image height down to 8 rather than 32. That routes the low-resolution U-Net levels onto the register-weight path instead of the generic or other routes. This routing change is active by default and risks worse occupancy on tiny images.

Measured after the change: 75.88 utterances/s. Within noise of the previous version (-0.2%).

```diff
diff --git a/diffusion-separation_amd/csrc/common.h b/diffusion-separation_amd/csrc/common.h
--- a/diffusion-separation_amd/csrc/common.h
+++ b/diffusion-separation_amd/csrc/common.h
@@ -214,12 +214,14 @@
 #define DS_OPT_NO_SW_ROWS4 32768u
 #define DS_OPT_SW_ROWS4 65536u
 #define DS_OPT_NO_SWS 16384u
+#define DS_OPT_NO_RW2 131072u
+#define DS_OPT_RW2_ALL 262144u
 #define DS_OPT_NO_WFRAG 32u
 unsigned ds_default_opts();
 int ds_num_cus();
 enum { DS_CLS_CONV_N64 = 0, DS_CLS_CONV_N32, DS_CLS_CONV_8X8, DS_CLS_GEMM_N64, DS_CLS_GEMM_N32, DS_CLS_GEMM_8X8, DS_CLS_WS,
        DS_CLS_SMALL, DS_CLS_RW, DS_CLS_ATTN, DS_CLS_SW, DS_CLS_SWS, DS_NCLS };
-enum class ConvRoute { GENERIC, WS, THIN_IN, THIN_OUT, SMALL, RW, SW, SWS };
+enum class ConvRoute { GENERIC, WS, THIN_IN, THIN_OUT, SMALL, RW, SW, SWS, RW2 };
 struct ConvPlan {
   ConvRoute route;
   int cls;
@@ -242,6 +244,9 @@
 }
 bool ds_conv_rw_supported(const ConvArgs& a);
 int ds_launch_conv_rw(const ConvArgs& a, hipStream_t st);
+int ds_rw_blocks_per_image(const ConvArgs& a, int tiles);
+bool ds_conv_rw2_supported(const ConvArgs& a);
+int ds_launch_conv_rw2(const ConvArgs& a, hipStream_t st);
 inline bool ds_sw_frag_shape(int taps, int Cin, int Cout) { return (Cout == 64 || Cout == 128 || Cout == 256) && Cin % 64 == 0 && Cin >= 64 && Cin <= 512; }
 bool ds_conv_sw_supported(const ConvArgs& a);
 int ds_launch_conv_sw(const ConvArgs& a, int rows, hipStream_t st);
diff --git a/diffusion-separation_amd/csrc/conv3x3_rw.hip b/diffusion-separation_amd/csrc/conv3x3_rw.hip
--- a/diffusion-separation_amd/csrc/conv3x3_rw.hip
+++ b/diffusion-separation_amd/csrc/conv3x3_rw.hip
@@ -753,11 +753,13 @@
 
 }
 
+int ds_rw_blocks_per_image(const ConvArgs& a, int tiles) { return rw_blocks_per_image(a, tiles); }
+
 bool ds_conv_rw_supported(const ConvArgs& a) {
   const int CO = a.Cout;
   if (!(a.dtype == DS_BF16 && a.taps == 9 && ((CO == 64 && (a.Cin == 64 || a.Cin == 128)) || (CO == 128 && a.Cin == 128)) &&
         a.w_bs == 0 && (a.w_chunked == 0 || a.w_chunked == 32) && a.bias_mode == 0 && !a.div_b && a.W % TW == 0 && a.H % 8 == 0 &&
-        a.H >= 32 && a.W >= 32 && a.ldy >= CO && a.ldy % 8 == 0 && (!a.res || (a.ldr >= CO && a.ldr % 8 == 0))))
+        a.H >= (CO == 64 ? 8 : 32) && a.W >= 32 && a.ldy >= CO && a.ldy % 8 == 0 && (!a.res || (a.ldr >= CO && a.ldr % 8 == 0))))
     return false;
   if (a.x2 ? !(a.C1 % KC == 0 && a.C1 > 0 && a.C1 < a.Cin && a.ldx % 8 == 0 && a.ldx2 % 8 == 0) : a.ldx % 8 != 0) return false;
   const bool gn = a.gn_scale || a.gn_acc1;
diff --git a/diffusion-separation_amd/csrc/conv3x3_rw2.hip b/diffusion-separation_amd/csrc/conv3x3_rw2.hip
--- /dev/null
+++ b/diffusion-separation_amd/csrc/conv3x3_rw2.hip
@@ -0,0 +1,748 @@
+#include <stdlib.h>
+
+#include "conv3x3_halo.h"
+
+namespace {
+
+constexpr int KC = 64;
+constexpr int NKB = KC / 16;
+constexpr int KSC = 9 * NKB;
+static_assert(KC * 2 + 16 == AROW && KC / 8 == PPL, "a pixel's chunk is one 128-byte line");
+
+struct RwK {
+  const bf16_t* x; long x_bs; int ldx; int C1;
+  const bf16_t* x2; long x2_bs; int ldx2;
+  const bf16_t* w; int w_chunked;
+  const bf16_t* wfrag; const bf16_t* swfrag;
+  const float* gn_scale; const float* gn_shift;
+  const long long* gn_acc1; const long long* gn_acc2; const float* gn_gamma; const float* gn_beta;
+  int gn_groups; float gn_inv_count; float gn_eps;
+  const float* bias; const float* bias_b; int bias_b_ld;
+  const bf16_t* res; long res_bs; int ldr;
+  float out_scale;
+  bf16_t* y; long y_bs; int ldy;
+  long long* stats;
+  const bf16_t* sx; long sx_bs; int ldsx; int sC1;
+  const bf16_t* sx2; long sx2_bs; int ldsx2;
+  const bf16_t* sw; int sw_chunked; int sw_shift; int sCin;
+  int H, W, G, tiles_x, tiles_per_img;
+  int dbg;
+};
+
+constexpr int NT2 = 512;
+constexpr int PASS = NT2 / PPL;
+
+#ifndef RW2_LDS_KS
+#ifdef DS_HALF_F16
+#define RW2_LDS_KS 12
+#else
+#define RW2_LDS_KS 20
+#endif
+#endif
+
+template <int NSK>
+struct Rw2Geom {
+  static constexpr int NCH = 1, NCG = 2, RPW = 2;
+  static constexpr int CO = 32 * NCG, PGN = 4;
+  static constexpr int TH = PGN * RPW, HH_ = TH + 2, HP = HH_ * HW_;
+  static constexpr int NI = TH * TW * PPL / NT2, NBP = HP - TH * TW, NB = (NBP * PPL + NT2 - 1) / NT2;
+  static constexpr int NL = NI + NB;
+  static_assert(PASS == 2 * TW && TH * TW * PPL % NT2 == 0, "one staging pass = two tile rows");
+  static constexpr int LDS_A = NL * PASS * AROW;
+  static constexpr int CIN = NCH * KC, SCIN = NSK * KC;
+  static constexpr int LDS_TAB = (2 * CIN + CO) * 4;
+  static constexpr int LDS_DESC = NB * NT2 * 4;
+  static_assert((NI + NB) * PASS >= HP + NB * PASS - NBP, "dummy pixels of the last border pass fit the slot");
+  static constexpr int NPH = NCH + NSK;
+  static constexpr int NKS = NCH * KSC + NSK * NKB;
+  static constexpr int NWL3 = RW2_LDS_KS + NSK * NKB <= 23 ? RW2_LDS_KS : 23 - NSK * NKB;
+  static constexpr int NWL = NWL3 + NSK * NKB, NWR = NKS - NWL;
+  static constexpr int LDS_WL = NWL * NCG * 64 * 16;
+  static constexpr int WL_STEP = NCG * 64 * 16;
+  static constexpr int OFF_TAB = 2 * LDS_A, OFF_WL = OFF_TAB + ((LDS_TAB + 15) & ~15), OFF_DESC = OFF_WL + LDS_WL;
+  static constexpr int LDS_TOTAL = OFF_DESC + LDS_DESC;
+  static constexpr int chunk_of(int P) { return P < NSK ? NCH + P : P - NSK; }
+  static_assert(LDS_TOTAL <= 160 * 1024, "LDS budget of one CU");
+  static_assert(NT2 * 36 * 4 <= LDS_TOTAL, "the statistics reduce reuses the block's LDS");
+};
+
+template <int NSK, int MODE>
+__global__ __launch_bounds__(NT2, 2) void conv3x3_rw2_kernel(RwK p) {
+  using G = Rw2Geom<NSK>;
+  constexpr int NCH = G::NCH, RPW = G::RPW, NCG = G::NCG;
+  constexpr int CO = G::CO, PGN = G::PGN;
+  constexpr int TH = G::TH, HP = G::HP, LDS_A = G::LDS_A, NL = G::NL, NPH = G::NPH, NKS = G::NKS, CIN = G::CIN, NWR = G::NWR;
+  extern __shared__ __attribute__((aligned(16))) char smem[];
+  char* sA = smem;
+  float* sTab = reinterpret_cast<float*>(smem + G::OFF_TAB);
+  int* sDesc = reinterpret_cast<int*>(smem + G::OFF_DESC);
+  const int tid = threadIdx.x;
+  const int lane = tid & 63, wave = __builtin_amdgcn_readfirstlane(tid >> 6);
+  const int l32 = lane & 31, h = lane >> 5;
+  const int cg = wave % NCG, pg = wave / NCG;
+  const int b = blockIdx.x / p.G, part = blockIdx.x % p.G;
+  const int t0 = (int)((long)part * p.tiles_per_img / p.G);
+  const int nt = (int)((long)(part + 1) * p.tiles_per_img / p.G) - t0;
+
+  static_assert(CIN <= NT2 && CO <= NT2, "one table entry per thread");
+  constexpr int CPG_MAX = 8;
+  long long t_s[CPG_MAX], t_q[CPG_MAX];
+  float t_gam = 1.f, t_bet = 0.f, t_sc = 1.f, t_sh = 0.f, t_bias = 0.f;
+#pragma unroll
+  for (int j = 0; j < CPG_MAX; ++j) { t_s[j] = 0; t_q[j] = 0; }
+  if (tid < CIN) {
+    const int c = tid;
+    if (p.gn_acc1) {
+      const int C1 = p.C1, C2 = CIN - C1;
+      const int cpg = CIN / p.gn_groups, g0 = (c / cpg) * cpg;
+#pragma unroll
+      for (int j = 0; j < CPG_MAX; ++j) {
+        if (j < cpg) {
+          const int cc = g0 + j;
+          const long long* src = cc < C1 ? p.gn_acc1 + ((long)b * C1 + cc) * 2 : p.gn_acc2 + ((long)b * C2 + (cc - C1)) * 2;
+          t_s[j] = src[0];
+          t_q[j] = src[1];
+        }
+      }
+      t_gam = p.gn_gamma ? p.gn_gamma[c] : 1.f;
+      t_bet = p.gn_beta ? p.gn_beta[c] : 0.f;
+    } else if (p.gn_scale) {
+      t_sc = p.gn_scale[(long)b * CIN + c];
+      t_sh = p.gn_shift[(long)b * CIN + c];
+    }
+  }
+  if (tid < CO) t_bias = (p.bias ? p.bias[tid] : 0.f) + (p.bias_b ? p.bias_b[(long)b * p.bias_b_ld + tid] : 0.f);
+  auto build_tables = [&]() __attribute__((always_inline)) {
+    if (tid < CIN) {
+      float sc = t_sc, sh = t_sh;
+      if (p.gn_acc1) {
+        long long t_ssum = 0, t_ssq = 0;
+#pragma unroll
+        for (int j = 0; j < CPG_MAX; ++j) { t_ssum += t_s[j]; t_ssq += t_q[j]; }
+        ds_gn_affine_from_acc(t_ssum, t_ssq, p.gn_inv_count, p.gn_eps, t_gam, t_bet, sc, sh);
+      }
+      sTab[tid] = sc;
+      sTab[CIN + tid] = sh;
+    }
+    if (tid < CO) sTab[2 * CIN + tid] = t_bias * p.out_scale;
+  };
+  const int slot = tid & (PPL - 1);
+  constexpr int NI = G::NI, NB = G::NB, NBP = G::NBP;
+  const int ixp = tid / PPL;
+  unsigned fl = 0;
+  int dstb[NB];
+#pragma unroll
+  for (int kb = 0; kb < NB; ++kb) {
+    const int bi = ixp + PASS * kb;
+    int hy, hx;
+    if (bi < HW_) { hy = 0; hx = bi; }
+    else if (bi < 2 * HW_) { hy = G::HH_ - 1; hx = bi - HW_; }
+    else if (bi < 2 * HW_ + TH) { hy = 1 + bi - 2 * HW_; hx = 0; }
+    else { hy = 1 + bi - 2 * HW_ - TH; hx = HW_ - 1; }
+    const bool in = bi < NBP;
+    const unsigned flg = in ? (hy == 0 ? 1u : 0u) | (hy == G::HH_ - 1 ? 2u : 0u) | (hx == 0 ? 4u : 0u) | (hx == HW_ - 1 ? 8u : 0u) : 16u;
+    sDesc[kb * NT2 + tid] = in ? (hy - 1) * p.W + (hx - 1) : 0;
+    dstb[kb] = (in ? hy * HW_ + hx : HP + (bi - NBP)) * AROW + slot * 16;
+    fl |= flg << (5 * kb);
+  }
+  const int iyp = ixp >> 5, ixc = ixp & 31;
+  const int ldi0 = ((1 + iyp) * HW_ + 1 + ixc) * AROW + slot * 16;
+  const int ipix = iyp * p.W + ixc;
+
+  const int M = p.H * p.W;
+  const __amdgpu_buffer_rsrc_t rx1 = rsrc(p.x + (long)b * p.x_bs, (unsigned)M * p.ldx * 2u);
+  const __amdgpu_buffer_rsrc_t rx2 = p.x2 ? rsrc(p.x2 + (long)b * p.x2_bs, (unsigned)M * p.ldx2 * 2u) : rx1;
+  const __amdgpu_buffer_rsrc_t rs1 = NSK ? rsrc(p.sx + (long)b * p.sx_bs, (unsigned)M * p.ldsx * 2u) : rx1;
+  const __amdgpu_buffer_rsrc_t rs2 = (NSK && p.sx2) ? rsrc(p.sx2 + (long)b * p.sx2_bs, (unsigned)M * p.ldsx2 * 2u) : rs1;
+  const __amdgpu_buffer_rsrc_t ry = rsrc(p.y + (long)b * p.y_bs, (unsigned)M * p.ldy * 2u);
+
+  u32x4_t wf[NWR > 0 ? NWR : 1];
+  char* sWl = smem + G::OFF_WL + (cg * 64 + lane) * 16;
+  auto put_w = [&](int ks, const u32x4_t& v) __attribute__((always_inline)) {
+    if (ks < NWR) wf[ks] = v;
+    else if (pg == 0) *reinterpret_cast<u32x4_t*>(sWl + (ks - NWR) * G::WL_STEP) = v;
+  };
+  auto load_weights = [&]() __attribute__((always_inline)) {
+    const bool wfm = p.wfrag != nullptr, sfm = NSK && p.swfrag != nullptr;
+    const __amdgpu_buffer_rsrc_t rw = rsrc(wfm ? p.wfrag : p.w, 9u * CO * CIN * 2u);
+    const __amdgpu_buffer_rsrc_t rsw = (NSK && p.sw) ? rsrc(sfm ? p.swfrag : p.sw, (unsigned)CO * G::SCIN * 2u) : rsrc(p.w, 0u);
+    const unsigned vfrag = (unsigned)((cg * 64 + lane) * 16);
+    const int co = cg * 32 + l32;
+    const bool wc = p.w_chunked != 0;
+    const unsigned vlane = wfm ? vfrag : (wc ? (unsigned)((co * 32 + h * 8) * 2) : (unsigned)((co * 9 * CIN + h * 8) * 2));
+    const bool sc_ = NSK && p.sw_chunked != 0;
+    const int kcs = sc_ ? p.sw_chunked : 16;
+    const unsigned vl2 = sfm ? vfrag : (sc_ ? (unsigned)((co * kcs + h * 8) * 2) : (unsigned)((co * G::SCIN + h * 8) * 2));
+    auto load_one = [&](int ks) __attribute__((always_inline)) {
+      if (ks < NCH * KSC) {
+        const int c = ks / KSC, tap = (ks % KSC) / NKB, kb = ks % NKB;
+        const int chb = c * KC + kb * 16;
+        const unsigned so = wfm ? (unsigned)(ks * NCG * 1024)
+                                : (wc ? (unsigned)((((chb >> 5) * 9 + tap) * CO * 32 + (chb & 31)) * 2) : (unsigned)((tap * CIN + chb) * 2));
+        put_w(ks, ld16v(rw, vlane, so));
+      } else {
+        const int chb = (ks - NCH * KSC) * 16;
+        const unsigned so = sfm ? (unsigned)((ks - NCH * KSC) * NCG * 1024)
+                                : (sc_ ? (unsigned)((((chb >> p.sw_shift) * CO) * kcs + (chb & (kcs - 1))) * 2) : (unsigned)(chb * 2));
+        u32x4_t f = ld16v(rsw, vl2, so);
+        if (!p.sw) {
+          const int d = co - (chb + 8 * h);
+#pragma unroll
+          for (int e = 0; e < 4; ++e) f[e] = d == 2 * e ? DS_H_ONE : (d == 2 * e + 1 ? DS_H_ONE << 16 : 0u);
+        }
+        put_w(ks, f);
+      }
+    };
+#pragma unroll
+    for (int ks = NWR; ks < NKS; ++ks) load_one(ks);
+#pragma unroll
+    for (int ks = 0; ks < NWR; ++ks) load_one(ks);
+  };
+
+  u32x4_t pa[NL];
+  struct TileG { int pix0; unsigned edge; };
+  auto geom_at = [&](int ty, int tx, bool valid) {
+    TileG g;
+    const int y0 = ty * TH, x0 = tx * TW;
+    g.edge = (y0 == 0 ? 1u : 0u) | (y0 + TH == p.H ? 2u : 0u) | (x0 == 0 ? 4u : 0u) | (x0 + TW == p.W ? 8u : 0u);
+    g.pix0 = valid ? y0 * p.W + x0 : 0x3fffff;
+    return g;
+  };
+  auto tile_geom = [&](int i) {
+    const int t = t0 + i;
+    const int ty = t / p.tiles_x;
+    return geom_at(ty, t - ty * p.tiles_x, i < nt);
+  };
+  auto piece_ok = [&](auto P_, const TileG& g, int k) __attribute__((always_inline)) {
+    constexpr int P = decltype(P_)::value;
+    const unsigned em = (P < NCH ? (g.edge | 16u) : 31u) << (5 * (k - NI));
+    return (fl & em) == 0u;
+  };
+  auto issue_one = [&](auto P_, const TileG& g, int k, int rel) __attribute__((always_inline)) {
+    constexpr int P = decltype(P_)::value;
+    constexpr bool CONV = P < NCH;
+    constexpr int CB = (CONV ? P : P - NCH) * KC;
+    const int c1 = CONV ? p.C1 : p.sC1;
+    const bool second = CB >= c1;
+    const unsigned ld2 = (unsigned)(CONV ? (second ? p.ldx2 : p.ldx) : (second ? p.ldsx2 : p.ldsx)) * 2u;
+    const unsigned co2 = (unsigned)((second ? CB - c1 : CB) * 2) + (unsigned)slot * 16u;
+    const __amdgpu_buffer_rsrc_t r = CONV ? (second ? rx2 : rx1) : (second ? rs2 : rs1);
+    if constexpr (!CONV) {
+      if (k >= NI) return;
+    }
+    if (k < NI) {
+      const unsigned off = __umul24((unsigned)(g.pix0 + 2 * k * p.W + ipix), ld2) + co2;
+      pa[k] = ld16v(r, off, 0);
+      return;
+    }
+    const unsigned off = __umul24((unsigned)(rel + g.pix0), ld2) + co2;
+    pa[k] = ld16v(r, piece_ok(P_, g, k) ? off : OOB, 0);
+  };
+  constexpr bool FOLD = MODE == 2 && NSK == 0;
+#if defined(DS_HALF_F16) && !defined(RW_ACT_F32)
+  constexpr bool ACT_PK = true;
+#else
+  constexpr bool ACT_PK = false;
+#endif
+  constexpr int PIPE_LAG = 2;
+  float gsc[ACT_PK ? 1 : 8], gsh[ACT_PK ? 1 : 8];
+  unsigned psc[ACT_PK ? 4 : 1], psh[ACT_PK ? 4 : 1];
+  auto act_tab = [&](int c) __attribute__((always_inline)) {
+    if constexpr (MODE != 0) {
+      const float4* ts = reinterpret_cast<const float4*>(sTab + c * KC + slot * 8);
+      const float4* th = reinterpret_cast<const float4*>(sTab + CIN + c * KC + slot * 8);
+      const float4 s0 = ts[0], s1 = ts[1], h0 = th[0], h1 = th[1];
+      float a[8] = {s0.x, s0.y, s0.z, s0.w, s1.x, s1.y, s1.z, s1.w}, b_[8] = {h0.x, h0.y, h0.z, h0.w, h1.x, h1.y, h1.z, h1.w};
+      if constexpr (FOLD) {
+#pragma unroll
+        for (int j = 0; j < 8; ++j) { a[j] *= -1.4426950408889634f; b_[j] *= -1.4426950408889634f; }
+      }
+      if constexpr (ACT_PK) {
+#pragma unroll
+        for (int d = 0; d < 4; ++d) { psc[d] = pack_h2(a[2 * d], a[2 * d + 1]); psh[d] = pack_h2(b_[2 * d], b_[2 * d + 1]); }
+      } else {
+#pragma unroll
+        for (int j = 0; j < 8; ++j) { gsc[j] = a[j]; gsh[j] = b_[j]; }
+      }
+    }
+  };
+  u32x4_t so;
+  float uz[3][2], ut[3][2];
+  unsigned uzp[3], utp[3], uxp[3], udp[3], urp[3];
+  auto unit_s01 = [&](auto P1_, int u0, int u1) __attribute__((always_inline)) {
+    constexpr int P1 = decltype(P1_)::value;
+    if constexpr (P1 < NCH && MODE != 0) {
+      const int q0 = u0 >= 0 ? u0 % 3 : 0, q1 = u1 >= 0 ? u1 % 3 : 0;
+      if constexpr (ACT_PK) {
+        unsigned z = 0, x = 0, e = 0, dd = 0, r = 0;
+        if (u0 >= 0) {
+          asm("v_pk_fma_f16 %0, %1, %2, %3" : "=v"(z) : "v"(pa[u0 >> 2][u0 & 3]), "v"(psc[u0 & 3]), "v"(psh[u0 & 3]));
+          x = z;
+          if constexpr (MODE == 2 && !FOLD) asm("v_pk_mul_f16 %0, %1, %2" : "=v"(x) : "v"(z), "s"(0xbdc5bdc5u));
+        }
+        if constexpr (MODE == 2) {
+          if (u1 >= 0) asm("v_pk_add_f16 %0, %1, %2" : "=v"(dd) : "v"(utp[q1]), "s"(0x3c003c00u));
+          if (u0 >= 0) asm("v_exp_f16 %0, %1" : "=v"(e) : "v"(x));
+          if (u1 >= 0) asm("v_rcp_f16 %0, %1" : "=v"(r) : "v"(dd));
+          if (u0 >= 0) asm("v_exp_f16_sdwa %0, %1 dst_sel:WORD_1 dst_unused:UNUSED_PRESERVE src0_sel:WORD_1" : "+v"(e) : "v"(x));
+          if (u1 >= 0) asm("v_rcp_f16_sdwa %0, %1 dst_sel:WORD_1 dst_unused:UNUSED_PRESERVE src0_sel:WORD_1" : "+v"(r) : "v"(dd));
+          if (u1 >= 0) urp[q1] = r;
+          if (u0 >= 0) utp[q0] = e;
+        }
+        if (u0 >= 0) uzp[q0] = z;
+      } else {
+        if (u1 >= 0 && MODE == 2) {
+          ut[q1][0] = __builtin_amdgcn_rcpf(1.0f + ut[q1][0]);
+          ut[q1][1] = __builtin_amdgcn_rcpf(1.0f + ut[q1][1]);
+        }
+        if (u0 >= 0) {
+          const unsigned w = pa[u0 >> 2][u0 & 3];
+          const int d = u0 & 3;
+          const float lo = h_lo(w), hi = h_hi(w);
+          const float z0 = fmaf(lo, gsc[2 * d], gsh[2 * d]), z1 = fmaf(hi, gsc[2 * d + 1], gsh[2 * d + 1]);
+          uz[q0][0] = z0; uz[q0][1] = z1;
+          if (MODE == 2) {
+            ut[q0][0] = __builtin_amdgcn_exp2f(FOLD ? z0 : z0 * -1.4426950408889634f);
+            ut[q0][1] = __builtin_amdgcn_exp2f(FOLD ? z1 : z1 * -1.4426950408889634f);
+          }
+        }
+      }
+    }
+  };
+  auto unit_s2x = [&](auto P1_, auto P2_, auto FIN_, const TileG& g1, const TileG& g2, int sl, int u, int rel) __attribute__((always_inline)) {
+    constexpr int P1 = decltype(P1_)::value;
+    constexpr bool FIN_ONLY = decltype(FIN_)::value;
+    const int k = u >> 2, d = u & 3, q = u % 3;
+    if constexpr (!FIN_ONLY) {
+    if constexpr (P1 < NCH && MODE != 0) {
+      if constexpr (ACT_PK) {
+        unsigned v = uzp[q];
+        if constexpr (MODE == 2) asm volatile("v_pk_mul_f16 %0, %1, %2" : "=v"(v) : "v"(uzp[q]), "v"(urp[q]));
+        so[d] = v;
+      } else {
+        float z0 = uz[q][0], z1 = uz[q][1];
+        if (MODE == 2) { z0 *= ut[q][0]; z1 *= ut[q][1]; }
+        so[d] = pack_h2(z0, z1);
+      }
+    } else {
+      so[d] = pa[k][d];
+    }
+    }
+    if (d == 3) {
+      if (P1 < NCH && MODE != 0 && k >= NI) {
+        const bool ok = piece_ok(P1_, g1, k);
+        so.x = ok ? so.x : 0u;
+        so.y = ok ? so.y : 0u;
+        so.z = ok ? so.z : 0u;
+        so.w = ok ? so.w : 0u;
+      }
+      if (P1 < NCH || k < NI)
+        *reinterpret_cast<u32x4_t*>(sA + sl * LDS_A + (k < NI ? ldi0 + k * 2 * HW_ * AROW : dstb[k < NI ? 0 : k - NI])) = so;
+      issue_one(P2_, g2, k, rel);
+    }
+  };
+  auto unit_s2 = [&](auto P1_, auto P2_, const TileG& g1, const TileG& g2, int sl, int u, int rel) __attribute__((always_inline)) {
+    unit_s2x(P1_, P2_, std::false_type{}, g1, g2, sl, u, rel);
+  };
+  auto unit_fin = [&](auto P1_, auto P2_, const TileG& g1, const TileG& g2, int sl, int u, int rel) __attribute__((always_inline)) {
+    unit_s2x(P1_, P2_, std::true_type{}, g1, g2, sl, u, rel);
+  };
+  auto unit = [&](auto P1_, auto P2_, const TileG& g1, const TileG& g2, int sl, int u, int rel) __attribute__((always_inline)) {
+    unit_s01(P1_, u, -1);
+    unit_s01(P1_, -1, u);
+    unit_s2(P1_, P2_, g1, g2, sl, u, rel);
+  };
+
+  f32x16 acc[RPW];
+#pragma unroll
+  for (int r = 0; r < RPW; ++r)
+#pragma unroll
+    for (int e = 0; e < 16; ++e) acc[r][e] = 0.f;
+  float ssum[16], ssq[16];
+#pragma unroll
+  for (int j = 0; j < 16; ++j) { ssum[j] = 0.f; ssq[j] = 0.f; }
+  const bool has_stats = p.stats != nullptr;
+  const float osc = FOLD ? p.out_scale * -0.6931471805599453f : p.out_scale;
+  const int fbase = (pg * RPW * HW_ + l32) * AROW + h * 16;
+
+  auto swap_halves = [&](u32x4_t& v) __attribute__((always_inline)) {
+    auto r0 = __builtin_amdgcn_permlane32_swap(v.x, v.z, false, false);
+    auto r1 = __builtin_amdgcn_permlane32_swap(v.y, v.w, false, false);
+    v.x = r0[0]; v.z = r0[1]; v.y = r1[0]; v.w = r1[1];
+  };
+  u32x4_t ov0;
+  const int srow = lane >> 4;
+  const unsigned spiece = (unsigned)(cg * 64 + (srow & 1) * 32 + (srow >> 1) * 16);
+  auto epi_unit = [&](const TileG& g, int r, int j, const float4& t0, const float4& t1) __attribute__((always_inline)) {
+    float v[8];
+    v[0] = fmaf(acc[r][8 * j + 0], osc, t0.x); v[1] = fmaf(acc[r][8 * j + 1], osc, t0.y);
+    v[2] = fmaf(acc[r][8 * j + 2], osc, t0.z); v[3] = fmaf(acc[r][8 * j + 3], osc, t0.w);
+    v[4] = fmaf(acc[r][8 * j + 4], osc, t1.x); v[5] = fmaf(acc[r][8 * j + 5], osc, t1.y);
+    v[6] = fmaf(acc[r][8 * j + 6], osc, t1.z); v[7] = fmaf(acc[r][8 * j + 7], osc, t1.w);
+#pragma unroll
+    for (int e = 0; e < 8; ++e) {
+      ssum[8 * j + e] += v[e];
+      ssq[8 * j + e] = fmaf(v[e], v[e], ssq[8 * j + e]);
+    }
+    u32x4_t ov = {pack_h2(v[0], v[1]), pack_h2(v[2], v[3]), pack_h2(v[4], v[5]), pack_h2(v[6], v[7])};
+    swap_halves(ov);
+    if (j == 0) {
+      ov0 = ov;
+    } else {
+      u32x4_t a = ov0, b2 = ov;
+#pragma unroll
+      for (int d = 0; d < 4; ++d) {
+        auto q = __builtin_amdgcn_permlane16_swap(a[d], b2[d], false, false);
+        a[d] = q[0]; b2[d] = q[1];
+      }
+      const int pix = g.pix0 + (pg * RPW + r) * p.W + (lane & 15);
+      const unsigned o = __umul24((unsigned)pix, (unsigned)p.ldy * 2u) + spiece;
+      const unsigned o1 = o, o2 = o + 16u * (unsigned)p.ldy * 2u;
+      __builtin_amdgcn_raw_buffer_store_b128(a, ry, o1, 0, 0);
+      __builtin_amdgcn_raw_buffer_store_b128(b2, ry, o2, 0, 0);
+    }
+  };
+  constexpr bool REL_REGS = NWR * 4 <= 176 || NCG == 4;
+#ifndef RW2_BIAS_REGS
+#define RW2_BIAS_REGS 0
+#endif
+  constexpr bool BIAS_REGS = RW2_BIAS_REGS;
+  float4 breg[2][2];
+  int relreg[G::NB];
+  auto epi_bias = [&](int j, float4& t0, float4& t1) __attribute__((always_inline)) {
+    if constexpr (BIAS_REGS) {
+      t0 = breg[j][0];
+      t1 = breg[j][1];
+    } else {
+      t0 = *reinterpret_cast<const float4*>(sTab + 2 * CIN + cg * 32 + 8 * (2 * j) + 4 * h);
+      t1 = *reinterpret_cast<const float4*>(sTab + 2 * CIN + cg * 32 + 8 * (2 * j + 1) + 4 * h);
+    }
+  };
+
+  constexpr int RH = RPW / 2;
+#ifndef RW2_W_E
+#define RW2_W_E 2
+#define RW2_W_N 5
+#endif
+  constexpr int W_E = RW2_W_E, W_N = RW2_W_N;
+  float et[2][2] = {{0.f, 0.f}, {0.f, 0.f}};
+  u32x4_t osa = {0, 0, 0, 0}, osb = {0, 0, 0, 0};
+  auto half = [&](auto P_, auto HF_, auto EPI_, int slot_r, const TileG& ge, const TileG& g1, const TileG& g2) __attribute__((always_inline)) {
+    constexpr int P = decltype(P_)::value, HF = decltype(HF_)::value;
+    constexpr bool EPI = decltype(EPI_)::value;
+    constexpr int C = G::chunk_of(P);
+    constexpr bool CONV = C < NCH;
+    constexpr int NK = CONV ? KSC : NKB;
+    constexpr int W0 = CONV ? C * KSC : NCH * KSC + (C - NCH) * NKB;
+    constexpr int C1 = G::chunk_of((P + 1) % NPH), C2 = G::chunk_of((P + 2) % NPH);
+    constexpr int NU = NL * 4;
+    constexpr bool ACT1 = C1 < NCH && MODE != 0;
+    constexpr int LAG = ACT1 ? PIPE_LAG : 0, NUV = NU + LAG, NLU = 2 * NUV;
+    constexpr int NGH = NK * RH;
+    constexpr int w0 = (P == 0) ? W_E : W_N, w1 = (P == NPH - 1) ? W_E : W_N, CAP = NGH * (w0 + w1);
+    auto lub = [](int GP) constexpr { return NLU * (GP <= NGH ? GP * w0 : NGH * w0 + (GP - NGH) * w1) / CAP; };
+    constexpr int NLE = RH * 22;
+    constexpr int R0 = HF * RH, ER0 = HF ? 0 : RH;
+    const char* fb = sA + slot_r * LDS_A + fbase + R0 * HW_ * AROW;
+    if constexpr (EPI) {
+#pragma unroll
+      for (int r = 0; r < RH; ++r) asm volatile("s_nop 11" : "+v"(acc[ER0 + r]));
+    }
+    if constexpr (HF == 0 && C1 < NCH) act_tab(C1);
+    constexpr int SUB = CONV ? 3 : 1, RFN = CONV ? RH + 2 : RH, NG = NK / SUB;
+    static_assert(SUB * RH >= RFN, "the next group's fragments are read in the MFMA slots of the current one");
+    auto ldg = [&](int g, int j) __attribute__((always_inline)) {
+      const int dx = CONV ? g / NKB : 1, kb = g % NKB, row = CONV ? j : j + 1;
+      return *reinterpret_cast<const u32x4_t*>(fb + (row * HW_ + dx) * AROW + kb * 32);
+    };
+    u32x4_t rf[2][RFN];
+#pragma unroll
+    for (int j = 0; j < RFN; ++j) rf[0][j] = ldg(0, j);
+    auto widx = [](int ks) {
+      if (!CONV) return ks;
+      const int g = ks / 3, dy = ks % 3, dx = g / NKB, kb = g % NKB;
+      return (dy * 3 + dx) * NKB + kb;
+    };
+#define RW_FRAG(ks, r) rf[((ks) / SUB) & 1][(r) + (CONV ? (ks) % SUB : 0)]
+#define RW_FRAG_LAST(ks) rf[((ks) / SUB) & 1][RFN - 1]
+    u32x4_t wl = {0, 0, 0, 0}, wln = {0, 0, 0, 0};
+    if constexpr (W0 + widx(0) >= NWR) wl = *reinterpret_cast<const u32x4_t*>(sWl + (W0 + widx(0) - NWR) * G::WL_STEP);
+    int rels[2][NL];
+    auto fetch_rels = [&](int ks, int par) __attribute__((always_inline)) {
+      const int gp0 = HF * NGH + ks * RH;
+#pragma unroll
+      for (int L = lub(gp0); L < lub(gp0 + RH); ++L) {
+        const int u = (L >> 1) - LAG;
+        if ((L & 1) && u >= 0 && u < NU && (u & 3) == 3 && (u >> 2) >= NI)
+          rels[par][u >> 2] = REL_REGS ? relreg[(u >> 2) - NI] : sDesc[((u >> 2) - NI) * NT2 + tid];
+      }
+    };
+    fetch_rels(0, 0);
+
+    auto unit_lump = [&](int L, int par) __attribute__((always_inline)) {
+      const int v = L >> 1;
+      const int u0 = v < NU ? v : -1, u1 = LAG ? ((v >= 1 && v - 1 < NU) ? v - 1 : -1) : v, u2 = v - LAG;
+      const bool s2 = u2 >= 0 && u2 < NU;
+      if ((L & 1) == 0) {
+        if constexpr (ACT1 && ACT_PK) {
+          if (u0 >= 0) {
+            asm volatile("v_pk_fma_f16 %0, %1, %2, %3" : "=v"(uzp[u0 % 3]) : "v"(pa[u0 >> 2][u0 & 3]), "v"(psc[u0 & 3]), "v"(psh[u0 & 3]));
+            if constexpr (MODE == 2 && !FOLD) asm volatile("v_pk_mul_f16 %0, %1, %2" : "=v"(uxp[u0 % 3]) : "v"(uzp[u0 % 3]), "s"(0xbdc5bdc5u));
+          }
+          if constexpr (MODE == 2) {
+            if (u1 >= 0) asm volatile("v_pk_add_f16 %0, %1, %2" : "=v"(udp[u1 % 3]) : "v"(utp[u1 % 3]), "s"(0x3c003c00u));
+            if (s2) asm volatile("v_pk_mul_f16 %0, %1, %2" : "=v"(so[u2 & 3]) : "v"(uzp[u2 % 3]), "v"(urp[u2 % 3]));
+            if (u0 >= 0) asm volatile("v_exp_f16 %0, %1" : "=v"(utp[u0 % 3]) : "v"(FOLD ? uzp[u0 % 3] : uxp[u0 % 3]));
+            if (u1 >= 0) asm volatile("v_rcp_f16 %0, %1" : "=v"(urp[u1 % 3]) : "v"(udp[u1 % 3]));
+          } else {
+            if (s2) so[u2 & 3] = uzp[u2 % 3];
+          }
+        } else if constexpr (ACT1) {
+          if (u0 >= 0) unit_s01(std::integral_constant<int, C1>{}, u0, -1);
+        }
+      } else {
+        if constexpr (ACT1 && ACT_PK) {
+          if constexpr (MODE == 2) {
+            if (u0 >= 0) asm volatile("v_exp_f16_sdwa %0, %1 dst_sel:WORD_1 dst_unused:UNUSED_PRESERVE src0_sel:WORD_1" : "+v"(utp[u0 % 3]) : "v"(FOLD ? uzp[u0 % 3] : uxp[u0 % 3]));
+            if (u1 >= 0) asm volatile("v_rcp_f16_sdwa %0, %1 dst_sel:WORD_1 dst_unused:UNUSED_PRESERVE src0_sel:WORD_1" : "+v"(urp[u1 % 3]) : "v"(udp[u1 % 3]));
+          }
+        } else if constexpr (ACT1) {
+          if (u1 >= 0) unit_s01(std::integral_constant<int, C1>{}, -1, u1);
+        }
+        if (s2) {
+          const int rel = ((u2 & 3) == 3 && (u2 >> 2) >= NI) ? rels[par][u2 >> 2] : 0;
+          if constexpr (ACT1 && ACT_PK) unit_fin(std::integral_constant<int, C1>{}, std::integral_constant<int, C2>{}, g1, g2, slot_r ^ 1, u2, rel);
+          else unit_s2(std::integral_constant<int, C1>{}, std::integral_constant<int, C2>{}, g1, g2, slot_r ^ 1, u2, rel);
+        }
+      }
+    };
+    auto epi_lump = [&](int LE) __attribute__((always_inline)) {
+      const int rr = ER0 + LE / 22, x = LE % 22;
+      if (x < 20) {
+        const int j = x / 10, y = x % 10;
+        const bool isA = y == 0 || y == 1 || y == 3 || y == 5 || y == 7;
+        const int pr = y == 0 ? 0 : (y == 1 ? 1 : (y == 2 ? 0 : (y == 3 ? 2 : (y == 4 ? 1 : (y == 5 ? 3 : (y == 6 ? 2 : (y == 7 ? 4 : 3)))))));
+        if (y == 9) {
+          if (j == 0) {
+            asm volatile("v_permlane32_swap_b32 %0, %1" : "+v"(osa[0]), "+v"(osa[2]));
+            asm volatile("v_permlane32_swap_b32 %0, %1" : "+v"(osa[1]), "+v"(osa[3]));
+          } else {
+            asm volatile("v_permlane32_swap_b32 %0, %1" : "+v"(osb[0]), "+v"(osb[2]));
+            asm volatile("v_permlane32_swap_b32 %0, %1" : "+v"(osb[1]), "+v"(osb[3]));
+          }
+        } else if (isA) {
+          if (pr < 4) {
+            const int e0 = 8 * j + 2 * pr;
+            float b0, b1;
+            if constexpr (BIAS_REGS) {
+              b0 = pr == 0 ? breg[j][0].x : (pr == 1 ? breg[j][0].z : (pr == 2 ? breg[j][1].x : breg[j][1].z));
+              b1 = pr == 0 ? breg[j][0].y : (pr == 1 ? breg[j][0].w : (pr == 2 ? breg[j][1].y : breg[j][1].w));
+            } else {
+              const float2 bb = *reinterpret_cast<const float2*>(sTab + 2 * CIN + cg * 32 + 8 * (2 * j + (pr >> 1)) + 4 * h + 2 * (pr & 1));
+              b0 = bb.x; b1 = bb.y;
+            }
+            asm volatile("v_fma_f32 %0, %1, %2, %3" : "=v"(et[pr & 1][0]) : "v"(acc[rr][e0]), "s"(osc), "v"(b0));
+            asm volatile("v_fma_f32 %0, %1, %2, %3" : "=v"(et[pr & 1][1]) : "v"(acc[rr][e0 + 1]), "s"(osc), "v"(b1));
+          }
+          if (pr >= 1) {
+            const int q = pr - 1;
+            if (j == 0) asm volatile(DS_CVT_PK_H_ASM " %0, %1, %2" : "=v"(osa[q]) : "v"(et[q & 1][0]), "v"(et[q & 1][1]));
+            else asm volatile(DS_CVT_PK_H_ASM " %0, %1, %2" : "=v"(osb[q]) : "v"(et[q & 1][0]), "v"(et[q & 1][1]));
+          }
+        } else {
+          const int e0 = 8 * j + 2 * pr;
+          asm volatile("v_add_f32 %0, %0, %1" : "+v"(ssum[e0]) : "v"(et[pr & 1][0]));
+          asm volatile("v_add_f32 %0, %0, %1" : "+v"(ssum[e0 + 1]) : "v"(et[pr & 1][1]));
+          asm volatile("v_fma_f32 %0, %1, %1, %0" : "+v"(ssq[e0]) : "v"(et[pr & 1][0]));
+          asm volatile("v_fma_f32 %0, %1, %1, %0" : "+v"(ssq[e0 + 1]) : "v"(et[pr & 1][1]));
+        }
+      } else if (x == 20) {
+#pragma unroll
+        for (int d = 0; d < 4; ++d) asm volatile("v_permlane16_swap_b32 %0, %1" : "+v"(osa[d]), "+v"(osb[d]));
+      } else {
+        const int pix = ge.pix0 + (pg * RPW + rr) * p.W + (lane & 15);
+        const unsigned o = __umul24((unsigned)pix, (unsigned)p.ldy * 2u) + spiece;
+        const unsigned o1 = o, o2 = o + 16u * (unsigned)p.ldy * 2u;
+        __builtin_amdgcn_raw_buffer_store_b128(osa, ry, o1, 0, 0);
+        __builtin_amdgcn_raw_buffer_store_b128(osb, ry, o2, 0, 0);
+      }
+    };
+
+#pragma unroll
+    for (int ks = 0; ks < NK; ++ks) {
+      if (ks + 1 < NK) fetch_rels(ks + 1, (ks + 1) & 1);
+      const int wi = W0 + widx(ks), win = W0 + widx(ks + 1 < NK ? ks + 1 : ks);
+      if (win >= NWR && ks + 1 < NK) wln = *reinterpret_cast<const u32x4_t*>(sWl + (win - NWR) * G::WL_STEP);
+      const u32x4_t wk = wi < NWR ? wf[wi < NWR ? wi : 0] : wl;
+#define RW_DEP , "v"(RW_FRAG_LAST(ks))
+#pragma unroll
+      for (int r = 0; r < RH; ++r) {
+        if (wi < NWR) {
+          if (P == 0 && ks == 0) asm volatile(DS_MFMA_H32_ASM " %0, %1, %2, 0" : "=v"(acc[R0 + r]) : "a"(wk), "v"(RW_FRAG(ks, r)) RW_DEP);
+          else asm volatile(DS_MFMA_H32_ASM " %0, %1, %2, %0" : "+v"(acc[R0 + r]) : "a"(wk), "v"(RW_FRAG(ks, r)) RW_DEP);
+        } else {
+          if (P == 0 && ks == 0) asm volatile(DS_MFMA_H32_ASM " %0, %1, %2, 0" : "=v"(acc[R0 + r]) : "v"(wk), "v"(RW_FRAG(ks, r)) RW_DEP);
+          else asm volatile(DS_MFMA_H32_ASM " %0, %1, %2, %0" : "+v"(acc[R0 + r]) : "v"(wk), "v"(RW_FRAG(ks, r)) RW_DEP);
+        }
+        {
+          const int g = ks / SUB, q = (ks % SUB) * RH + r;
+          if (q < RFN && g + 1 < NG) rf[(g + 1) & 1][q] = ldg(g + 1, q);
+        }
+        const int gh = ks * RH + r, gp = HF * NGH + gh;
+#pragma unroll
+        for (int L = lub(gp); L < lub(gp + 1); ++L) unit_lump(L, ks & 1);
+        if constexpr (EPI) {
+#pragma unroll
+          for (int LE = gh * NLE / NGH; LE < (gh + 1) * NLE / NGH; ++LE) epi_lump(LE);
+        }
+      }
+      wl = wln;
+      __builtin_amdgcn_sched_barrier(0);
+    }
+  };
+
+  TileG gc = tile_geom(0);
+  constexpr int CH0 = G::chunk_of(0), CH1 = G::chunk_of(1 % NPH);
+  const TileG g1st = NPH > 1 ? gc : tile_geom(1);
+  {
+#pragma unroll
+    for (int k = 0; k < NL; ++k) issue_one(std::integral_constant<int, CH0>{}, gc, k, k < NI ? 0 : sDesc[(k < NI ? 0 : k - NI) * NT2 + tid]);
+    load_weights();
+    build_tables();
+    sync_lds();
+    if constexpr (REL_REGS) {
+#pragma unroll
+      for (int k = 0; k < NB; ++k) relreg[k] = sDesc[k * NT2 + tid];
+    }
+    if constexpr (BIAS_REGS) {
+#pragma unroll
+      for (int j = 0; j < 2; ++j) {
+        breg[j][0] = *reinterpret_cast<const float4*>(sTab + 2 * CIN + cg * 32 + 8 * (2 * j) + 4 * h);
+        breg[j][1] = *reinterpret_cast<const float4*>(sTab + 2 * CIN + cg * 32 + 8 * (2 * j + 1) + 4 * h);
+      }
+    }
+    act_tab(CH0);
+#pragma unroll
+    for (int u = 0; u < NL * 4; ++u)
+      unit(std::integral_constant<int, CH0>{}, std::integral_constant<int, CH1>{}, gc, g1st, 0, u,
+           (u >> 2) < NI ? 0 : sDesc[((u >> 2) < NI ? 0 : (u >> 2) - NI) * NT2 + tid]);
+  }
+  if (wave >= 4) __builtin_amdgcn_s_setprio(1);
+  TileG gp = tile_geom(nt);
+  int ph = 0;
+  TileG gnc = tile_geom(1);
+  int ty2 = (t0 + 2) / p.tiles_x, tx2 = (t0 + 2) - ty2 * p.tiles_x;
+  for (int i = 0; i < nt; ++i) {
+    const TileG gn = gnc, gnn = geom_at(ty2, tx2, i + 2 < nt);
+    auto run = [&](auto self, auto P_) __attribute__((always_inline)) {
+      constexpr int P = decltype(P_)::value;
+      sync_lds();
+      const int slot_r = ph & 1;
+      half(P_, std::integral_constant<int, 0>{}, std::integral_constant<bool, P == 0>{}, slot_r, gp, ((P + 1) / NPH == 0 ? gc : gn), ((P + 2) / NPH == 0 ? gc : ((P + 2) / NPH == 1 ? gn : gnn)));
+      if constexpr (P == 0) {
+        if (i == 0) {
+#pragma unroll
+          for (int j = 0; j < 16; ++j) { ssum[j] = 0.f; ssq[j] = 0.f; }
+        }
+      }
+      half(P_, std::integral_constant<int, 1>{}, std::integral_constant<bool, P == NPH - 1>{}, slot_r, gc, ((P + 1) / NPH == 0 ? gc : gn), ((P + 2) / NPH == 0 ? gc : ((P + 2) / NPH == 1 ? gn : gnn)));
+      ++ph;
+      if constexpr (P + 1 < NPH) self(self, std::integral_constant<int, P + 1>{});
+    };
+    run(run, std::integral_constant<int, 0>{});
+    gp = gc;
+    gc = gn;
+    gnc = gnn;
+    if (++tx2 == p.tiles_x) { tx2 = 0; ++ty2; }
+  }
+#pragma unroll
+  for (int r = 0; r < RH; ++r) asm volatile("s_nop 11" : "+v"(acc[RH + r]));
+#pragma unroll
+  for (int e = 0; e < RH * 2; ++e) {
+    float4 t0, t1;
+    epi_bias(e & 1, t0, t1);
+    epi_unit(gp, RH + (e >> 1), e & 1, t0, t1);
+  }
+  if (has_stats) {
+    __syncthreads();
+    float* red = reinterpret_cast<float*>(smem);
+    constexpr int RED_ROW = 36;
+#pragma unroll
+    for (int q = 0; q < 4; ++q) {
+      *reinterpret_cast<float4*>(red + tid * RED_ROW + 4 * q) = make_float4(ssum[4 * q], ssum[4 * q + 1], ssum[4 * q + 2], ssum[4 * q + 3]);
+      *reinterpret_cast<float4*>(red + tid * RED_ROW + 16 + 4 * q) = make_float4(ssq[4 * q], ssq[4 * q + 1], ssq[4 * q + 2], ssq[4 * q + 3]);
+    }
+    __syncthreads();
+    if (tid < 2 * CO) {
+      const int co = tid >> 1, st = tid & 1;
+      const int wcg = co >> 5, c32 = co & 31, q = c32 >> 3, hh = (c32 >> 2) & 1, i = c32 & 3;
+      double a = 0.0;
+      for (int wpg = 0; wpg < PGN; ++wpg)
+        for (int l = 0; l < 32; ++l) {
+          const int t = (wpg * NCG + wcg) * 64 + hh * 32 + l;
+          a += (double)red[t * RED_ROW + st * 16 + 4 * q + i];
+        }
+      ds_stat_flush(p.stats + ((long)b * CO + co) * 2, st, a);
+    }
+  }
+}
+
+
+template <int NSK, int MODE>
+int rw2_launch(const RwK& k0, const ConvArgs& a, hipStream_t st) {
+  using G = Rw2Geom<NSK>;
+  RwK k = k0;
+  const int tiles = (a.H / G::TH) * (a.W / TW);
+  k.G = ds_rw_blocks_per_image(a, tiles);
+  k.tiles_x = a.W / TW;
+  k.tiles_per_img = tiles;
+  auto kern = conv3x3_rw2_kernel<NSK, MODE>;
+  DS_FUNC_LDS_ONCE(kern, G::LDS_TOTAL);
+  hipLaunchKernelGGL(kern, dim3(a.B * k.G), dim3(NT2), G::LDS_TOTAL, st, k);
+  DS_LAUNCH_CHECK();
+  {
+    static char name[64] = {0};
+    if (!name[0]) snprintf(name, sizeof(name), "conv3x3_rw2_kernel<%d,%d>", NSK, MODE);
+    ds_set_last_conv_kernel(name);
+  }
+  return 0;
+}
+
+}
+
+bool ds_conv_rw2_supported(const ConvArgs& a) {
+  return a.Cout == 64 && a.Cin == 64 && !a.x2 && (!a.sx || a.sCin == 64) && ds_conv_rw_supported(a);
+}
+
+int ds_launch_conv_rw2(const ConvArgs& a, hipStream_t st) {
+  RwK k;
+  k.x = reinterpret_cast<const bf16_t*>(a.x); k.x_bs = a.x_bs; k.ldx = a.ldx; k.C1 = a.x2 ? a.C1 : a.Cin;
+  k.x2 = reinterpret_cast<const bf16_t*>(a.x2); k.x2_bs = a.x2_bs; k.ldx2 = a.x2 ? a.ldx2 : a.ldx;
+  k.w = reinterpret_cast<const bf16_t*>(a.w); k.w_chunked = a.w_chunked;
+  k.wfrag = reinterpret_cast<const bf16_t*>(a.w_frag);
+  k.swfrag = (a.sx && a.sw) ? reinterpret_cast<const bf16_t*>(a.sw_frag) : nullptr;
+  k.gn_scale = a.gn_scale; k.gn_shift = a.gn_shift;
+  k.gn_acc1 = a.gn_acc1; k.gn_acc2 = a.gn_acc2; k.gn_gamma = a.gn_gamma; k.gn_beta = a.gn_beta;
+  k.gn_groups = a.gn_groups; k.gn_inv_count = a.gn_inv_count; k.gn_eps = a.gn_eps;
+  k.bias = a.bias; k.bias_b = a.bias_b; k.bias_b_ld = a.bias_b_ld;
+  k.res = reinterpret_cast<const bf16_t*>(a.res); k.res_bs = a.res_bs; k.ldr = a.ldr;
+  k.out_scale = a.out_scale;
+  k.y = reinterpret_cast<bf16_t*>(a.y); k.y_bs = a.y_bs; k.ldy = a.ldy;
+  k.stats = a.stats_acc;
+  k.sx = reinterpret_cast<const bf16_t*>(a.sx); k.sx_bs = a.sx_bs; k.ldsx = a.ldsx; k.sC1 = a.sx2 ? a.sC1 : a.sCin;
+  k.sx2 = reinterpret_cast<const bf16_t*>(a.sx2); k.sx2_bs = a.sx2_bs; k.ldsx2 = a.sx2 ? a.ldsx2 : a.ldsx;
+  k.sw = reinterpret_cast<const bf16_t*>(a.sw); k.sw_chunked = a.sw_chunked; k.sw_shift = a.sw_chunked ? __builtin_ctz(a.sw_chunked) : 0;
+  k.sCin = a.sCin;
+  k.H = a.H; k.W = a.W; k.G = 0; k.tiles_x = 0; k.tiles_per_img = 0;
+  k.dbg = 0;
+  if (a.res) {
+    k.sx = reinterpret_cast<const bf16_t*>(a.res); k.sx_bs = a.res_bs; k.ldsx = a.ldr; k.sC1 = a.Cout;
+    k.sx2 = nullptr; k.sx2_bs = 0; k.ldsx2 = a.ldr; k.sw = nullptr; k.sw_chunked = 0; k.sw_shift = 0; k.sCin = a.Cout;
+  }
+  const int mode = ((a.gn_scale || a.gn_acc1) && a.gn_act) ? 2 : 0;
+  const int nsk = a.sx ? a.sCin / KC : (a.res ? a.Cout / KC : 0);
+#define RW2_GO(NSK_) return mode == 2 ? rw2_launch<NSK_, 2>(k, a, st) : rw2_launch<NSK_, 0>(k, a, st)
+  if (nsk == 0) RW2_GO(0);
+  RW2_GO(1);
+#undef RW2_GO
+}
diff --git a/diffusion-separation_amd/csrc/conv_mfma.hip b/diffusion-separation_amd/csrc/conv_mfma.hip
--- a/diffusion-separation_amd/csrc/conv_mfma.hip
+++ b/diffusion-separation_amd/csrc/conv_mfma.hip
@@ -800,6 +800,7 @@
   return taps == 9 ? 32 : 64;
 }
 
+constexpr bool RW2_DEFAULT = false;
 ConvPlan ds_conv_plan(const ConvArgs& a) {
   const unsigned o = a.opts;
   const bool any_size = o & DS_OPT_RW_SMALL;
@@ -823,7 +824,11 @@
                                    : rows && !(rows == 4 && (o & DS_OPT_NO_SW_ROWS4)) && (!p.rw_ok || (!(o & DS_OPT_NO_SW_RW) && t8 < 2 * cus));
     if (take && !(o & DS_OPT_NO_SW)) return routed(ConvRoute::SW, DS_CLS_SW);
   }
-  if (p.rw_ok) return routed(ConvRoute::RW, DS_CLS_RW);
+  if (p.rw_ok) {
+    if (!(o & DS_OPT_NO_RW2) && ds_conv_rw2_supported(a) && ((o & DS_OPT_RW2_ALL) || (RW2_DEFAULT && a.H >= 128)))
+      return routed(ConvRoute::RW2, DS_CLS_RW);
+    return routed(ConvRoute::RW, DS_CLS_RW);
+  }
   if (ds_conv_ws_supported(a)) return routed(ConvRoute::WS, DS_CLS_WS);
   if (ds_conv_thin_in_supported(a)) return routed(ConvRoute::THIN_IN, DS_CLS_WS);
   if (ds_conv_thin_out_supported(a)) return routed(ConvRoute::THIN_OUT, DS_CLS_WS);
@@ -855,6 +860,7 @@
     case ConvRoute::SWS: return ds_launch_conv_sws(a, st);
     case ConvRoute::SW: return ds_launch_conv_sw(a, p.sw_rows, st);
     case ConvRoute::RW: return ds_launch_conv_rw(a, st);
+    case ConvRoute::RW2: return ds_launch_conv_rw2(a, st);
     case ConvRoute::WS: return ds_launch_conv_ws(a, st);
     case ConvRoute::THIN_IN: return ds_launch_conv_thin_in(a, st);
     case ConvRoute::THIN_OUT: return ds_launch_conv_thin_out(a, st);
diff --git a/diffusion-separation_amd/csrc/engine.hip b/diffusion-separation_amd/csrc/engine.hip
--- a/diffusion-separation_amd/csrc/engine.hip
+++ b/diffusion-separation_amd/csrc/engine.hip
@@ -16,6 +16,8 @@
     {"no_rw128", "DIFFSEP_NO_RW128", DS_OPT_NO_RW128},
     {"rw_small", "DIFFSEP_RW_SMALL", DS_OPT_RW_SMALL},
     {"no_rw_res", "DIFFSEP_NO_RW_RES", DS_OPT_NO_RW_RES},
+    {"no_rw2", nullptr, DS_OPT_NO_RW2},
+    {"rw2_all", nullptr, DS_OPT_RW2_ALL},
     {"no_wfrag", nullptr, DS_OPT_NO_WFRAG},
     {"no_attn_fused", nullptr, DS_OPT_NO_ATTN_FUSED},
     {"no_stft_fused", "DIFFSEP_NO_STFT_FUSED", DS_OPT_NO_STFT_FUSED},
```
